# wangchen615/kubernetes-simulator

Measured on AMD Instinct MI355X. Metric: pod-node Filter+Score evals/sec and pods bound/sec at 50k nodes, 1-8 GPUs, higher is better.
Workload: dtype int64; 1 GPU; C3: 50k nodes w/ taints+labels, 1M-pod trace, Filter(fit+taint+selector) -> Score(LR+BA) -> argmax -> bind, 1 pod/tick; nodes=50000, trace_pods=5570560, parallelism=single-gpu, batch_pods=192

## Files before the change

go/kubesim/engine/engine.go:

```go
package engine

import "C"

import (
	"runtime"
	"unsafe"

	"github.com/cpuguy83/strongerrors"
	"github.com/pkg/errors"
)

var ErrOutOfDomain = errors.New("outside the engine's exact domain")

type Engine struct {
	h *C.ks_engine
	n int
}

func status(e *Engine, rc C.ks_status) error {
	msg := ""
	if e != nil && e.h != nil {
		msg = C.GoString(C.ks_last_error(e.h))
	}
	switch rc {
	case C.KS_OK:
		return nil
	case C.KS_ENOTFOUND:
		return strongerrors.NotFound(errors.New(msg))
	case C.KS_EINVAL:
		return strongerrors.InvalidArgument(errors.New(msg))
	case C.KS_ERANGE:
		return errors.Wrap(ErrOutOfDomain, msg)
	default:
		return errors.Errorf("ks_engine: device error (%d): %s", int(rc), msg)
	}
}

const (
	ScorerConst          = C.KS_SCORER_CONST
	ScorerLeastRequested = C.KS_SCORER_LEAST_REQUESTED
	ScorerBalanced       = C.KS_SCORER_BALANCED
)

const (
	FilterFit      = uint32(C.KS_FILTER_FIT)
	FilterTaint    = uint32(C.KS_FILTER_TAINT)
	FilterSelector = uint32(C.KS_FILTER_SELECTOR)
)

const (
	FlagNoOverlap   = uint32(C.KS_ENGINE_NO_OVERLAP)
	FlagPrunedLists = uint32(C.KS_ENGINE_PRUNED_LISTS)
)

type ScorerSpec struct {
	Kind, Weight, Value int32
}

type Config struct {
	TickSeconds int
	FeedsScore  bool
	Filters     uint32
	Scorers     []ScorerSpec
	Device      int
	BatchPods   int
	EngineFlags uint32
}

func (c Config) toC() (C.ks_config, error) {
	var cfg C.ks_config
	if len(c.Scorers) > 8 {
		return cfg, strongerrors.InvalidArgument(errors.New("at most 8 scorers"))
	}
	cfg.abi_version = C.KS_ABI_VERSION
	cfg.tick_seconds = C.int32_t(c.TickSeconds)
	if c.FeedsScore {
		cfg.filter_mode = C.KS_FILTER_FEEDS_SCORE
	}
	cfg.filters = C.uint32_t(c.Filters)
	cfg.n_scorers = C.int32_t(len(c.Scorers))
	for i, s := range c.Scorers {
		cfg.scorers[i].kind = C.int32_t(s.Kind)
		cfg.scorers[i].weight = C.int32_t(s.Weight)
		cfg.scorers[i].value = C.int32_t(s.Value)
	}
	cfg.device = C.int32_t(c.Device)
	cfg.batch_pods = C.int32_t(c.BatchPods)
	cfg.engine_flags = C.uint32_t(c.EngineFlags)
	return cfg, nil
}

func New(c Config) (*Engine, error) {
	cfg, err := c.toC()
	if err != nil {
		return nil, err
	}
	e := &Engine{}
	if rc := C.ks_create(&cfg, &e.h); rc != C.KS_OK {
		return nil, errors.Errorf("ks_create rejected the configuration (%d)", int(rc))
	}
	runtime.SetFinalizer(e, (*Engine).Close)
	return e, nil
}

func (e *Engine) Close() {
	if e.h != nil {
		C.ks_destroy(e.h)
		e.h = nil
	}
	runtime.SetFinalizer(e, nil)
}

func CommUniqueID() ([]byte, error) {
	id := make([]byte, C.KS_COMM_ID_BYTES)
	if rc := C.ks_comm_unique_id((*C.uint8_t)(unsafe.Pointer(&id[0]))); rc != C.KS_OK {
		return nil, status(nil, rc)
	}
	return id, nil
}

func (e *Engine) Shard(world, rank int, id []byte, vshards int) error {
	defer runtime.KeepAlive(e)
	if len(id) != C.KS_COMM_ID_BYTES {
		return errors.Errorf("communicator id: %d bytes, want %d", len(id), C.KS_COMM_ID_BYTES)
	}
	rc := C.ks_shard(e.h, C.int32_t(world), C.int32_t(rank), (*C.uint8_t)(unsafe.Pointer(&id[0])), C.int32_t(vshards))
	return status(e, rc)
}

func (e *Engine) LoadNodes(alloc []int64, taint, label []uint64) error {
	defer runtime.KeepAlive(e)
	n := len(taint)
	if len(alloc) != 4*n || len(label) != n {
		return strongerrors.InvalidArgument(errors.New("LoadNodes: alloc must hold 4 values per node"))
	}
	if n == 0 {
		return status(e, C.ks_load_nodes(e.h, 0, nil, nil, nil))
	}
	err := status(e, C.ks_load_nodes(e.h, C.int64_t(n), (*C.int64_t)(unsafe.Pointer(&alloc[0])),
		(*C.uint64_t)(unsafe.Pointer(&taint[0])), (*C.uint64_t)(unsafe.Pointer(&label[0]))))
	if err == nil {
		e.n = n
	}
	return err
}

type Pods struct {
	Arrival  []int64
	Req      []int64
	KeyMask  []uint8
	Tol, Sel []uint64
	PhaseOff []int32
	PhaseSec []int32
	PhaseUse []int64
	Flags    []uint8
	Key      []int64
}

func i64p(s []int64) *C.int64_t {
	if len(s) == 0 {
		return nil
	}
	return (*C.int64_t)(unsafe.Pointer(&s[0]))
}
func u64p(s []uint64) *C.uint64_t {
	if len(s) == 0 {
		return nil
	}
	return (*C.uint64_t)(unsafe.Pointer(&s[0]))
}
func i32p(s []int32) *C.int32_t {
	if len(s) == 0 {
		return nil
	}
	return (*C.int32_t)(unsafe.Pointer(&s[0]))
}
func u8p(s []uint8) *C.uint8_t {
	if len(s) == 0 {
		return nil
	}
	return (*C.uint8_t)(unsafe.Pointer(&s[0]))
}

func (e *Engine) SubmitPods(p *Pods) error {
	defer runtime.KeepAlive(e)
	m := len(p.Arrival)
	if m == 0 {
		return nil
	}
	if len(p.Req) != 3*m || len(p.KeyMask) != m || len(p.Tol) != m || len(p.Sel) != m ||
		len(p.PhaseOff) != m+1 || len(p.Flags) != m || len(p.Key) != m ||
		int(p.PhaseOff[m]) > len(p.PhaseSec) || 3*int(p.PhaseOff[m]) > len(p.PhaseUse) {
		return strongerrors.InvalidArgument(errors.New("SubmitPods: inconsistent array lengths"))
	}
	return status(e, C.ks_submit_pods(e.h, C.int64_t(m), i64p(p.Arrival), i64p(p.Req), u8p(p.KeyMask),
		u64p(p.Tol), u64p(p.Sel), i32p(p.PhaseOff), i32p(p.PhaseSec), i64p(p.PhaseUse), u8p(p.Flags),
		i64p(p.Key)))
}

type Bind struct {
	Pod    int64
	Node   int32
	Status int32
	Tick   int64
}
// ... 140 lines not shown
```

include/ks_engine.h:

```cpp
#ifndef KS_ENGINE_H
#define KS_ENGINE_H
#include <stdint.h>

#ifdef __cplusplus
extern "C" {
#endif

#define KS_ABI_VERSION 2

typedef enum {
    KS_OK = 0,
    KS_EINVAL = 1,
    KS_ENOTFOUND = 2,
    KS_EDEVICE = 3,
    KS_ENOMEM = 4,
    KS_ERANGE = 5,
} ks_status;

enum { KS_FILTER_REFERENCE_LITERAL = 0, KS_FILTER_FEEDS_SCORE = 1 };
enum { KS_FILTER_FIT = 1, KS_FILTER_TAINT = 2, KS_FILTER_SELECTOR = 4 };
enum { KS_SCORER_CONST = 0, KS_SCORER_LEAST_REQUESTED = 1, KS_SCORER_BALANCED = 2 };
enum { KS_POD_OK = 0, KS_POD_OVER_CAPACITY = 1 };
enum { KS_PODFLAG_BAD_KEY = 1, KS_PODFLAG_BAD_SPEC = 2 };

typedef struct {
    int32_t kind;
    int32_t weight;
    int32_t value;
} ks_scorer;

typedef struct {
    int32_t abi_version;
    int32_t tick_seconds;
    int32_t filter_mode;
    uint32_t filters;
    int32_t n_scorers;
    ks_scorer scorers[8];
    int32_t device;
    int32_t batch_pods;
    uint32_t engine_flags;
    int32_t reserved[7];
} ks_config;

enum { KS_ENGINE_FORCE_WIDE = 1, KS_ENGINE_NO_TINY = 2, KS_ENGINE_NO_MICRO = 4,
       KS_ENGINE_ONE_POD_RESOLVER = 8, KS_ENGINE_CHUNK_RESOLVER = 64, KS_ENGINE_NO_OVERLAP = 256,
       KS_ENGINE_PRUNED_LISTS = 512 };

typedef struct {
    int64_t pod;
    int32_t node;
    int32_t status;
    int64_t tick;
} ks_bind;

typedef struct ks_engine ks_engine;

ks_status ks_create(const ks_config* cfg, ks_engine** out);
void ks_destroy(ks_engine* eng);

typedef struct ks_group ks_group;
ks_status ks_group_create(int32_t device, int32_t max_scenarios, ks_group** out);
void ks_group_destroy(ks_group* g);
ks_status ks_group_add(ks_group* g, const ks_config* cfg, ks_engine** out);
int32_t ks_group_size(const ks_group* g);

ks_status ks_shard_layout(int64_t n_nodes, int32_t world, int32_t vshards, int32_t* part_lo_out);
ks_status ks_merge_candidates(const uint64_t* cand_all, int32_t parts, int32_t B, uint64_t* out);
#define KS_COMM_ID_BYTES 128
ks_status ks_comm_unique_id(uint8_t* id_out );
ks_status ks_shard(ks_engine* eng, int32_t world, int32_t rank, const uint8_t* id, int32_t vshards);
typedef ks_status (*ks_allgather_fn)(void* user, int32_t rank, int32_t world, void* buf, int64_t bytes_per_rank);
ks_status ks_shard_host(ks_engine* eng, int32_t world, int32_t rank, int32_t vshards, ks_allgather_fn fn,
                        void* user);

ks_status ks_load_nodes(ks_engine* eng, int64_t n, const int64_t* alloc, const uint64_t* taint,
                        const uint64_t* label);

ks_status ks_submit_pods(ks_engine* eng, int64_t m, const int64_t* arrival_tick,
                         const int64_t* req, const uint8_t* keymask, const uint64_t* tol,
                         const uint64_t* sel, const int32_t* phase_off, const int32_t* phase_sec,
                         const int64_t* phase_use, const uint8_t* flags, const int64_t* key_id);

ks_status ks_step(ks_engine* eng, int64_t ticks, ks_bind* out, int64_t cap, int64_t* n_out);

ks_status ks_filter(ks_engine* eng, int64_t pod, uint8_t* mask_out);
ks_status ks_score(ks_engine* eng, int64_t pod, int64_t* score_out);

ks_status ks_usage(ks_engine* eng, int64_t* usage_out);

ks_status ks_usage_at(ks_engine* eng, int64_t t, int64_t* usage_out);

ks_status ks_usage_digest(ks_engine* eng, int64_t t_lo, int64_t t_hi, uint64_t* out);
uint64_t ks_node_mix(int64_t node);

ks_status ks_requested_at(ks_engine* eng, int64_t t, int64_t* out);
ks_status ks_filter_at(ks_engine* eng, int64_t pod, uint8_t* mask_out);
ks_status ks_score_at(ks_engine* eng, int64_t pod, int64_t* score_out);
#define KS_SERIES_COLS 7
ks_status ks_cluster_series(ks_engine* eng, int64_t t_lo, int64_t t_hi, int64_t* out);
ks_status ks_node_peaks(ks_engine* eng, int64_t t_lo, int64_t t_hi, int64_t* out);

ks_status ks_pod_lookup(ks_engine* eng, int32_t node, int64_t key_id, int64_t* pod_out);
ks_status ks_node_pods(ks_engine* eng, int32_t node, int64_t* pods_out, int64_t cap, int64_t* n_out);

enum { KS_PHASE_PENDING = 0, KS_PHASE_RUNNING = 1, KS_PHASE_SUCCEEDED = 2, KS_PHASE_FAILED = 3 };
typedef struct {
    int32_t phase;
    int32_t node;
    int64_t start_tick;
    int32_t total_seconds;
    int32_t pad;
} ks_pod_info;
ks_status ks_pod_status(ks_engine* eng, int64_t pod_lo, int64_t n, ks_pod_info* out);

int64_t ks_current_tick(const ks_engine* eng);
int32_t ks_tick_seconds(const ks_engine* eng);
int64_t ks_queued_pods(const ks_engine* eng);
const char* ks_last_error(const ks_engine* eng);

typedef struct {
    double step_ms;
    double scan_ms;
    double resolve_ms;
    int64_t launches;
    int64_t pods;
    double other_ms;
} ks_step_stats;
ks_status ks_last_step_stats(const ks_engine* eng, ks_step_stats* out);
typedef struct {
    double prep_ms, scan_ms, merge_ms, resolve_ms, fused_ms, part_ms, xchg_ms;
    int64_t prep_n, scan_n, merge_n, resolve_n, fused_n, xchg_n;
    double side_scan_ms, side_part_ms, side_xchg_ms, wait_ms;
    int64_t side_n;
    double usage_ms;
    int64_t usage_n, usage_pods;
} ks_kernel_stats;
ks_status ks_last_step_kernels(const ks_engine* eng, ks_kernel_stats* out);
ks_status ks_group_step(ks_group* g, int64_t ticks, ks_bind* out, int64_t cap, int64_t* n_out,
                        int32_t* status_out, ks_step_stats* stats);
ks_status ks_debug_counters(ks_engine* eng, int64_t* out32);
ks_status ks_debug_invariants(ks_engine* eng, int64_t* out4);
ks_status ks_debug_window(ks_engine* eng, void* out, int64_t cap, int64_t* size_out);
ks_status ks_debug_watch(ks_engine* eng, int64_t pod);
enum { KS_SELFTEST_LR_MICRO = 0 };
ks_status ks_selftest(int32_t device, int32_t test, int64_t* failures);
void ks_set_profiling(ks_engine* eng, int enable);
const char* ks_build_id(void);

#ifdef __cplusplus
}
#endif
#endif
```

kubernetes-simulator_amd/csrc/ks_cand.hip:

```cpp
#include <climits>

#include "ks_device.h"
#include "ks_prep.h"
#include "ks_scan.h"

namespace ks {
namespace sq {

constexpr int kR = kChR;
constexpr int kPrepThreads = 1024;
constexpr int kClBuf = 256;
static_assert(kR <= kWave, "one candidate per lane");
static_assert(kWinSlots <= kPrepThreads, "one window slot per prep thread");

__device__ __forceinline__ int32_t key_node(uint64_t key) { return (int32_t)(0xFFFFFFFFu - (uint32_t)key); }
__device__ __forceinline__ int32_t clamp32(int64_t v) { return (int32_t)(v > INT_MAX ? INT_MAX : v); }

template <typename T>
__device__ __forceinline__ const __attribute__((address_space(1))) T* cg(const T* p) {
    return (const __attribute__((address_space(1))) T*)p;
}

__global__ __launch_bounds__(kPrepThreads) void window_prep_kernel(const EngineArgs* __restrict__ A, int head, int spec,
                                                                    int slot) {
    const EngineArgs& a = A[0];
    __shared__ prep::PrepLDS L;
    prep::prep_body<kPrepThreads>(a, a.ctr[kCtrStart], a.ctr[kCtrEnd], a.ctr[kCtrErr], head, spec, slot, L);
}

#ifdef KS_MCL_DIAG
#define MDG_AT(I, T)                                                                      \
    do {                                                                                  \
        const uint64_t t_ = prep::pstamp();                                               \
        if (threadIdx.x == 0) atomicAdd((unsigned long long*)&a.ctr[(I)], t_ - (T));      \
        (T) = t_;                                                                         \
    } while (0)
using prep::pstamp;
#endif
constexpr int kRecWords = 12;
static_assert(kRecWords <= kRecDw, "record size");
constexpr int kSlotPending = -2;
static_assert(kSlotIds <= 65535, "slot ids in 16 bits");

__device__ __forceinline__ void put_rec(uint32_t* o, const NodeV& v) {
    o[0] = (uint32_t)v.ac; o[1] = (uint32_t)v.am; o[2] = (uint32_t)v.ag;
    o[3] = (uint32_t)clamp32(v.ap);
    o[4] = (uint32_t)v.rc; o[5] = (uint32_t)v.rm; o[6] = (uint32_t)v.rg;
    o[7] = (uint32_t)v.nr;
    o[8] = (uint32_t)v.taint; o[9] = (uint32_t)(v.taint >> 32); o[10] = (uint32_t)v.label; o[11] = (uint32_t)(v.label >> 32);
}

constexpr int kEPer = kEMax / 256;

static_assert(kTopLOverlap >= kTopL, "merged lists kept at the longest list length");
template <int kMode, int kLL>
__device__ __forceinline__ void cand_list(const EngineArgs& a, WinWS& ws, int i, const uint64_t* cand,
                                          const uint64_t* ek, int n_e) {
    static_assert(kLL >= kTopL && kLL <= kWave, "one list entry per lane");
    const int tid = threadIdx.x;
    PDG(uint64_t pt = pstamp();)
    __shared__ uint64_t buf[kClBuf];
    __shared__ int cnt;
    __shared__ uint64_t s_thr;
    __shared__ int s_full;
    if (tid == 0) cnt = 0;
    __syncthreads();
    if (tid < kWave) {
        const int lane = tid;
        const uint64_t x = lane < kLL ? cand[lane] : 0ull;
        const bool un = x != 0 && a.e_idx[key_node(x)] < 0;
        const uint64_t um = __ballot(un);
        const int rank = __popcll(um & ((1ull << lane) - 1ull));
        if (un && rank < kTopL) {
            const int pos = atomicAdd(&cnt, 1);
            if (pos < kClBuf) buf[pos] = x;
        }
        const uint64_t last = cand[kLL - 1];
        const bool enough = __popcll(um) >= kTopL;
        if (enough && un && rank == kTopL - 1) s_thr = x;
        if (!enough && lane == 0) s_thr = last != 0 ? last : 1ull;
        if (lane == 0) s_full = enough || last != 0;
    }
    __syncthreads();
    PDG(MDG_AT(9, pt);)
    const uint64_t thr = s_thr;
    const bool full = s_full != 0;
    for (int k = tid; k < n_e; k += blockDim.x)
        if (ek[k] != 0 && ek[k] >= thr) {
            const int pos = atomicAdd(&cnt, 1);
            if (pos < kClBuf) buf[pos] = ek[k];
        }
    __syncthreads();
    PDG(MDG_AT(10, pt);)
    const int c = cnt, n = c < kClBuf ? c : kClBuf;
    __shared__ uint64_t kept[kR];
    if (tid < n) {
        const uint64_t me = buf[tid];
        int r = 0;
        for (int u = 0; u < n; ++u) r += buf[u] > me;
        if (r < kR) kept[r] = me;
    }
    __syncthreads();
    PDG(MDG_AT(11, pt);)
    if (tid < kWave) {
        const int lane = tid;
        const bool valid = lane < (n < kR ? n : kR);
        const uint64_t me = valid ? kept[lane] : 0ull;
        const int32_t nd = key_node(me);
        NodeV rec{};
        int32_t eix = -1;
        if (valid) { rec = load_node(a.s, nd); eix = a.e_idx[nd]; }
        if (valid && a.det_cids) atomicMin(&a.n_first[nd], i * kR + lane);
        int sl = valid ? atomicCAS(&a.n_slot[nd], -1, kSlotPending) : 0;
        const bool claim = valid && sl == -1;
        const uint64_t cm = __ballot(claim);
        int base = 0;
        if (cm) {
            const int first = __ffsll((unsigned long long)cm) - 1;
            if (lane == first) base = atomicAdd(&ws.nslot, __popcll(cm));
            base = __shfl(base, first);
        }
        if (claim) {
            sl = base + __popcll(cm & ((1ull << lane) - 1ull));
            ws.slot_node[sl] = nd;
            if (sl < kSlotMax) {
                put_rec(ws.slot_rec[sl], rec);
                ws.slot_eix[sl] = eix;
            }
            atomicExch(&a.n_slot[nd], sl);
        }
        bool wait = valid && sl == kSlotPending;
        while (__ballot(wait)) {
            if (wait) {
                sl = __hip_atomic_load(&a.n_slot[nd], __ATOMIC_RELAXED, __HIP_MEMORY_SCOPE_AGENT);
                wait = sl < 0;
            }
            if (__ballot(wait)) __builtin_amdgcn_s_sleep(1);
        }
        if (valid) {
            ws.cl_key[i][lane] = me;
            ws.cl_slot[i][lane] = sl;
        }
    }
    PDG(__syncthreads(); MDG_AT(12, pt);)
    if (tid == 0) {
        ws.cl_info[i] = (c < kR ? c : kR) | (c > kR ? kClTrunc : 0) | (full ? kClFull : 0) | (c > kClBuf ? kClOvf : 0);
        ws.cl_thr[i] = thr;
    }
}

constexpr int kMergeMaxWaves = 16;
}
#ifdef KS_MCL_BYVAL
thread_local const EngineArgs* ks_mcl_host_args = nullptr;
#endif
namespace sq {
template <int kMode, int kLL>
#ifdef KS_MCL_BYVAL
__global__ __launch_bounds__(1024) void merge_cl_kernel(const EngineArgs av, const uint64_t* src,
                                                         int64_t pod_stride, int32_t nl, int64_t list_stride, int own_fb) {
    const EngineArgs& a = av;
#else
__global__ __launch_bounds__(1024) void merge_cl_kernel(const EngineArgs* __restrict__ A, const uint64_t* src,
                                                         int64_t pod_stride, int32_t nl, int64_t list_stride, int own_fb) {
    const EngineArgs& a = A[0];
#endif
    WinWS& ws = *a.sw;
    const bool own = src == nullptr || (own_fb && ws.rescan);
    if (own) {
        src = a.lists;
        pod_stride = (int64_t)a.nblk * kLL;
        nl = a.nblk;
        list_stride = kLL;
    }
    const int b = blockIdx.x;
    const int tid = threadIdx.x, lane = tid & 63, wave = tid >> 6;
    const int nthr = blockDim.x, nwav = nthr / kWave;
    const bool prn = a.lbit != nullptr;
    const int lset = prn ? ws.lset : 1;
    const bool pruned = own && prn;
    const int nbw = ws.nb, split = ws.split, moff = ws.moff, mpar = ws.mpar;
    const bool reuse = b < split;
    const int sb = b - split;
    __shared__ scn::FlagLDS F;
    int nfl = reuse ? 0 : nl;
    if (b < nbw && !reuse && pruned) nfl = scn::flagged_index(lbit_of(a, lset, sb), 0, nl, F);
    if (prn) {
        const int cs = b < split ? nbw - split + b : (b < nbw ? sb : b);
        for (int w = tid; w < 2 * a.nwl; w += nthr) lbit_of(a, w / a.nwl, cs)[w % a.nwl] = 0;
        if (tid < 2 * kThrCopies) *lthr_of(a, tid / kThrCopies, tid % kThrCopies, cs) = 0;
    }
    if (b >= nbw) return;
    PDG(uint64_t pt = pstamp(); if (tid == 0) atomicAdd((unsigned long long*)&a.ctr[5], 1ull);)
    uint64_t top[kLL];
#pragma unroll
    for (int k = 0; k < kLL; ++k) top[k] = 0;
    const uint64_t* lists = src + (int64_t)(reuse ? 0 : sb) * pod_stride;
    uint64_t lv0[kLL];
    const bool has0 = tid < nfl;
    {
        const int l0 = has0 ? (pruned ? scn::flagged_block(tid, 0, nl, F) : tid) : 0;
        const ulonglong2* lp = reinterpret_cast<const ulonglong2*>(lists + (int64_t)l0 * list_stride);
#pragma unroll
        for (int k = 0; k < kLL / 2; ++k) {
            const ulonglong2 w = has0 ? lp[k] : make_ulonglong2(0, 0);
            lv0[2 * k] = w.x;
            lv0[2 * k + 1] = w.y;
        }
    }
    __shared__ uint64_t ek[kEMax];
    const int n_e = ws.n_e;
    {
        const int64_t start = a.ctr[kCtrStart];
        const int hi = ws.win_hi[b], n_es = ws.n_es;
        uint4 er[2][3];
        int32_t en[2], eu[2], ue[2];
#pragma unroll
        for (int q = 0; q < 2; ++q) {
            const int k = tid + q * nthr;
            const int kc = k < kEMax ? k : kEMax - 1;
            const int ks = k < kWinSlots ? k : kWinSlots;
            en[q] = ws.e_node[kc];
            const uint4* r = reinterpret_cast<const uint4*>(ws.e_rec[kc]);
            er[q][0] = r[0]; er[q][1] = r[1]; er[q][2] = r[2];
            eu[q] = ws.e_off[ks];
            ue[q] = ws.e_off[ks < kWinSlots ? ks + 1 : ks];
        }
#if defined(KS_MCL_DIAG) && KS_MCL_DIAG == 2
        asm volatile("s_waitcnt vmcnt(0) lgkmcnt(0)" ::: "memory");
        uint64_t t_e0 = pstamp();
        if (tid == 0) atomicAdd((unsigned long long*)&a.ctr[13], t_e0 - pt);
#endif
        const PodRec p = a.pods[start + b];
#pragma unroll
        for (int q = 0; q < 2; ++q) {
            const int k = tid + q * nthr;
            if (k >= n_e) continue;
            NodeV v = get_rec12(er[q]);
            if (k < n_es) {
                for (int u = eu[q]; u < ue[q]; ++u) {
                    const int x = ws.e_slot[u];
                    if (x >= hi) break;
                    v.rc -= ws.ex_req[x][0]; v.rm -= ws.ex_req[x][1]; v.rg -= ws.ex_req[x][2]; v.nr -= 1;
                }
            }
            ek[k] = make_key(eval_t<kMode>(a.c, p, v), (uint32_t)en[q]);
        }
#pragma unroll 1
        for (int k = tid + 2 * nthr; k < n_e; k += nthr) {
            const int32_t n = ws.e_node[k];
            const uint4* r = reinterpret_cast<const uint4*>(ws.e_rec[k]);
            const uint4 w3[3] = {r[0], r[1], r[2]};
            NodeV w = get_rec12(w3);
            const int ue1 = k < n_es ? ws.e_off[k + 1] : 0;
            for (int u = k < n_es ? ws.e_off[k] : 0; u < ue1; ++u) {
                const int x = ws.e_slot[u];
                if (x >= hi) break;
                w.rc -= ws.ex_req[x][0]; w.rm -= ws.ex_req[x][1]; w.rg -= ws.ex_req[x][2]; w.nr -= 1;
            }
            ek[k] = make_key(eval_t<kMode>(a.c, p, w), (uint32_t)n);
        }
#if defined(KS_MCL_DIAG) && KS_MCL_DIAG == 2
        asm volatile("s_waitcnt vmcnt(0) lgkmcnt(0)" ::: "memory");
        if (tid == 0) { atomicAdd((unsigned long long*)&a.ctr[14], pstamp() - t_e0); atomicAdd((unsigned long long*)&a.ctr[24], (unsigned long long)(n_e > tid) + (n_e > tid + nthr)); }
        if (tid == 0) atomicAdd((unsigned long long*)&a.ctr[25], (unsigned long long)n_e);
#endif
    }
    if (has0) {
#pragma unroll
        for (int k = 0; k < kLL; ++k) top[k] = lv0[k];
    }
    for (int j = tid + nthr; j < nfl; j += nthr) {
        const int blk = pruned ? scn::flagged_block(j, 0, nl, F) : j;
        const ulonglong2* lp = reinterpret_cast<const ulonglong2*>(lists + (int64_t)blk * list_stride);
        uint64_t lv[kLL];
#pragma unroll
        for (int k = 0; k < kLL / 2; ++k) {
            const ulonglong2 w = lp[k];
            lv[2 * k] = w.x;
            lv[2 * k + 1] = w.y;
        }
        topl_insert<kLL>(top, lv);
    }
    __shared__ uint64_t wl[kMergeMaxWaves][kLL];
    __shared__ uint64_t pc[kLL];
    PDG(MDG_AT(6, pt);)
    int head = 0;
    for (int r = 0; r < kLL; ++r) {
        uint64_t h = 0;
#pragma unroll
        for (int k = 0; k < kLL; ++k) h = (k == head) ? top[k] : h;
        const uint64_t m = wave_max_u64(h);
        const uint64_t hit = __ballot(h == m && m != 0);
        if (lane == 0) wl[wave][r] = m;
        if (hit && lane == __ffsll((unsigned long long)hit) - 1) head++;
    }
    __syncthreads();
    PDG(MDG_AT(7, pt);)
    if (wave == 0 && nthr <= 256) {
        static_assert(4 * kLL <= kWave, "one candidate per lane");
        uint64_t v = lane < nwav * kLL ? wl[lane / kLL][lane % kLL] : 0ull;
        for (int r = 0; r < kLL; ++r) {
            const uint64_t m = wave_max_u64(v);
            if (lane == 0) pc[r] = m;
            if (m == 0) continue;
            const uint64_t h = __ballot(v == m);
            if (lane == __ffsll((unsigned long long)h) - 1) v = 0;
        }
    } else if (wave == 0) {
        constexpr int kPer = (kMergeMaxWaves * kLL + kWave - 1) / kWave;
        const int nc = nwav * kLL;
        uint64_t v[kPer];
#pragma unroll
        for (int q = 0; q < kPer; ++q) {
            const int c = lane + q * kWave;
            v[q] = c < nc ? wl[c / kLL][c % kLL] : 0ull;
        }
        for (int r = 0; r < kLL; ++r) {
            uint64_t lm = v[0];
#pragma unroll
            for (int q = 1; q < kPer; ++q) lm = lm > v[q] ? lm : v[q];
            const uint64_t m = wave_max_u64(lm);
            if (lane == 0) pc[r] = m;
            if (m == 0) continue;
            bool done = false;
#pragma unroll
            for (int q = 0; q < kPer; ++q) {
                const uint64_t h = __ballot(!done && v[q] == m);
                if (h && lane == __ffsll((unsigned long long)h) - 1) v[q] = 0;
                done = done || h != 0;
            }
        }
    }
    __syncthreads();
    if (reuse && tid < kLL) pc[tid] = ws.mrg[mpar ^ 1][b + moff][tid];
    if (reuse) __syncthreads();
    if (tid < kLL) ws.mrg[mpar][b][tid] = pc[tid];
    PDG(MDG_AT(8, pt);)
    cand_list<kMode, kLL>(a, ws, b, pc, ek, n_e);
}

}

hipError_t launch_window_prep(const EngineArgs* d, bool head, bool spec, int slot, hipStream_t st) {
    hipLaunchKernelGGL(sq::window_prep_kernel, dim3(1), dim3(sq::kPrepThreads), 0, st, d, head ? 1 : 0, spec ? 1 : 0,
                       slot & 1);
    return hipGetLastError();
}

hipError_t launch_merge_cl(const EngineArgs* d, int mode, int B, const uint64_t* lists, int64_t pod_stride,
                           int32_t nl, int64_t list_stride, int nl_max, hipStream_t st, int L, bool own_fallback) {
    const int fb = own_fallback ? 1 : 0;
    static_assert(sq::kEPer * 256 >= kEMax, "E keys per thread at 256 threads");
    const dim3 g(B), t(nl_max > 1024 ? 1024 : 256);
#ifdef KS_MCL_BYVAL
    if (!ks_mcl_host_args) return hipErrorInvalidValue;
    const EngineArgs hv = *ks_mcl_host_args;
#define d hv
#endif
#define KS_MCL(LL)                                                                                                   \
    switch (mode) {                                                                                                  \
        case kEvalMicro: hipLaunchKernelGGL((sq::merge_cl_kernel<kEvalMicro, LL>), g, t, 0, st, d, lists, pod_stride, nl, list_stride, fb); break; \
        case kEvalTiny: hipLaunchKernelGGL((sq::merge_cl_kernel<kEvalTiny, LL>), g, t, 0, st, d, lists, pod_stride, nl, list_stride, fb); break;   \
        case kEvalNarrow: hipLaunchKernelGGL((sq::merge_cl_kernel<kEvalNarrow, LL>), g, t, 0, st, d, lists, pod_stride, nl, list_stride, fb); break; \
        default: hipLaunchKernelGGL((sq::merge_cl_kernel<kEvalWide, LL>), g, t, 0, st, d, lists, pod_stride, nl, list_stride, fb); break;          \
    }
    if (L == kTopL) { KS_MCL(kTopL) }
    else if (L == kTopLOverlap) { KS_MCL(kTopLOverlap) }
    else return hipErrorInvalidValue;
#undef KS_MCL
#ifdef KS_MCL_BYVAL
#undef d
#endif
    return hipGetLastError();
}

}
```

kubernetes-simulator_amd/csrc/ks_device.h:

```cpp
#pragma once
#include <hip/hip_runtime.h>
#include <stdint.h>

namespace ks {

constexpr int kWave = 64;
constexpr int kTopL = 8;
#ifndef KS_OVERLAP_LIST
#define KS_OVERLAP_LIST 12
#endif
constexpr int kTopLOverlap = KS_OVERLAP_LIST;
static_assert(kTopLOverlap >= kTopL && kTopLOverlap <= 16 && kTopLOverlap % 2 == 0, "overlap list length");

enum : uint32_t { kFilterFit = 1, kFilterTaint = 2, kFilterSelector = 4 };

struct Cfg {
    int32_t n_nodes;
    int32_t nwb;
    int32_t filter_feeds;
    uint32_t filters;
    int32_t has_scorers;
    int32_t w_lr;
    int32_t w_ba;
    int32_t const_total;
// ... 392 lines not shown

enum : int { kEvalWide = 0, kEvalNarrow = 1, kEvalTiny = 2, kEvalMicro = 3 };

template <int kMode, class NS>
__host__ __device__ __forceinline__ uint32_t eval_t(const Cfg& c, const PodRec& p, const NS& n) {
    if constexpr (kMode == kEvalMicro) return eval_total1_micro(c, p, n);
    else if constexpr (kMode == kEvalTiny) return eval_total1_tiny(c, p, n);
    else if constexpr (kMode == kEvalNarrow) return eval_total1_narrow(c, p, n);
    else return eval_total1(c, p, n);
}

constexpr float kBoundLR = 1.5e-5f;
constexpr float kBoundBA = 3.0e-5f;
struct PruneF {
    float bc, ic, bm, im;
    int32_t live;
};
template <class NS>
__host__ __device__ __forceinline__ PruneF prune_prep(const Cfg& c, const NS& n) {
    PruneF f;
    f.ic = n.ac > 0 ? rcp_est((float)n.ac) : 0.f;
    f.bc = n.ac > 0 ? (float)(int64_t)(n.ac - n.rc) * f.ic : -1.f;
    f.im = n.am > 0 ? rcp_est((float)n.am) : 0.f;
    f.bm = n.am > 0 ? (float)(int64_t)(n.am - n.rm) * f.im : -1.f;
    f.live = c.has_scorers && !(c.filter_feeds && (c.filters & kFilterFit) && n.nr >= n.ap);
    return f;
}
template <int kMode, class NS>
__host__ __device__ __forceinline__ PruneF prune_prep_t(const Cfg& c, const NS& n) {
    if constexpr (kMode >= kEvalNarrow) {
        const int32_t ac = (int32_t)n.ac, am = (int32_t)n.am;
        PruneF f;
        f.ic = ac > 0 ? rcp_est((float)ac) : 0.f;
        f.bc = ac > 0 ? (float)(ac - (int32_t)n.rc) * f.ic : -1.f;
        f.im = am > 0 ? rcp_est((float)am) : 0.f;
        f.bm = am > 0 ? (float)(am - (int32_t)n.rm) * f.im : -1.f;
        f.live = c.has_scorers && !(c.filter_feeds && (c.filters & kFilterFit) && n.nr >= n.ap);
        return f;
    } else {
        return prune_prep(c, n);
    }
}
__host__ __device__ __forceinline__ uint32_t prune_tmax(const Cfg& c, const PruneF& f, float qc, float qm) {
    const float fc = fmaf(-qc, f.ic, f.bc), fm = fmaf(-qm, f.im, f.bm);
    int32_t total = c.const_total;
    const int32_t lc = fc > -kBoundLR ? (int32_t)(10.f * fc + kBoundLR) : 0;
    const int32_t lm = fm > -kBoundLR ? (int32_t)(10.f * fm + kBoundLR) : 0;
    total += c.w_lr * ((lc + lm) >> 1);
    if (fc > -kBoundLR && fm > -kBoundLR)
        total += c.w_ba * (int32_t)(10.f - 10.f * fabsf(fc - fm) + kBoundBA);
    return (uint32_t)total;
}

template <typename T>
__device__ __forceinline__ T sload(const T* p) {
    static_assert(sizeof(T) % 4 == 0, "sload: dword-sized types only");
    typedef const __attribute__((address_space(4))) uint32_t* cp;
    const cp q = (cp)p;
    T v;
    uint32_t* d = reinterpret_cast<uint32_t*>(&v);
#pragma unroll
    for (int i = 0; i < (int)(sizeof(T) / 4); ++i) d[i] = q[i];
    return v;
}

template <typename T>
__device__ __forceinline__ __attribute__((address_space(1))) T* gptr(T* p) {
    return (__attribute__((address_space(1))) T*)p;
}

__host__ __device__ __forceinline__ uint64_t make_key(uint32_t total1, uint32_t node) {
    return total1 ? (((uint64_t)total1 << 32) | (uint64_t)(0xFFFFFFFFu - node)) : 0ull;
}

template <int L = kTopL>
__host__ __device__ __forceinline__ void topl_insert(uint64_t (&top)[L], const uint64_t (&lv)[L]) {
#pragma unroll
    for (int k = 0; k < L; ++k) {
        uint64_t v = lv[k];
        if (v <= top[L - 1]) break;
#pragma unroll
        for (int s = 0; s < L; ++s) {
            const uint64_t t = top[s];
            const bool gt = v > t;
            top[s] = gt ? v : t;
            v = gt ? t : v;
        }
    }
}

__device__ __forceinline__ uint32_t dpp_max_step(uint32_t v, uint32_t w) { return v > w ? v : w; }
__device__ __forceinline__ uint32_t wave_max_u32(uint32_t v) {
    v = dpp_max_step(v, (uint32_t)__builtin_amdgcn_update_dpp(0, (int)v, 0x111, 0xf, 0xf, false));
    v = dpp_max_step(v, (uint32_t)__builtin_amdgcn_update_dpp(0, (int)v, 0x112, 0xf, 0xf, false));
    v = dpp_max_step(v, (uint32_t)__builtin_amdgcn_update_dpp(0, (int)v, 0x114, 0xf, 0xf, false));
    v = dpp_max_step(v, (uint32_t)__builtin_amdgcn_update_dpp(0, (int)v, 0x118, 0xf, 0xf, false));
    v = dpp_max_step(v, (uint32_t)__builtin_amdgcn_update_dpp((int)v, (int)v, 0x142, 0xa, 0xf, false));
    v = dpp_max_step(v, (uint32_t)__builtin_amdgcn_update_dpp((int)v, (int)v, 0x143, 0xc, 0xf, false));
    return (uint32_t)__builtin_amdgcn_readlane((int)v, 63);
}

__device__ __forceinline__ uint64_t wave_max_u64(uint64_t v) {
    const uint32_t hi = (uint32_t)(v >> 32), lo = (uint32_t)v;
    const uint32_t mh = wave_max_u32(hi);
    const uint32_t ml = wave_max_u32(hi == mh ? lo : 0u);
    return ((uint64_t)mh << 32) | ml;
}

enum : int64_t { kCtrStart = 0, kCtrEnd = 1, kCtrErr = 2, kCtrErrPod = 3, kCtrEarly = 4, kCtrRescan = 5, kCtrReuse = 6 };
enum : uint32_t { kFlagBadKey = 1, kFlagBadSpec = 2 };
enum : int64_t { kErrEinval = 1, kErrNotFound = 2 };

constexpr int kWinMaxB = 256;
constexpr int kWinSlots = 512;
#ifndef KS_CHR
#define KS_CHR 20
#endif
constexpr int kChR = KS_CHR;
constexpr int kRecDw = 20;
constexpr int kSlotMax = 1536;
constexpr int kSlotIds = kWinMaxB * kChR;
constexpr int32_t kNoFirst = 0x7F7F7F7F;
constexpr int kEMax = 2048;
constexpr int kTouchMax = kWinMaxB + kWinSlots;
constexpr int kSpecStride = 8;
constexpr int kSpecPrev = 3;
enum : int32_t { kClTrunc = 1 << 8, kClFull = 1 << 9, kClOvf = 1 << 10 };
struct WinWS {
    int32_t nb, e_cnt, n_e, n_es;
    int32_t win_hi[kWinMaxB];
    int32_t own[kWinMaxB];
    int32_t ex_q[kWinSlots];
    int32_t ex_ok[kWinSlots];
    int64_t ex_req[kWinSlots][3];
    int32_t e_node[kEMax];
    int32_t e_off[kWinSlots + 1];
    int32_t e_slot[kWinSlots];
    uint32_t e_rec[kEMax][12];
    uint64_t cl_key[kWinMaxB][kChR];
    int32_t cl_info[kWinMaxB];
    uint64_t cl_thr[kWinMaxB];
    int32_t cl_slot[kWinMaxB][kChR];
    int32_t nslot;
    int32_t nslot_hw;
#ifdef KS_SLOT_IDS_LEGACY
    int32_t slot_node[kSlotMax];
#else
    int32_t slot_node[kSlotIds];
#endif
    int32_t slot_eix[kSlotMax];
    uint32_t slot_rec[kSlotMax][kRecDw];
    int32_t touched[kTouchMax];
    int32_t n_touched, rescan;
    int32_t lset, pad_;
    int32_t split, moff, mpar, pad2_;
    uint64_t mrg[2][kWinMaxB][kTopLOverlap];
#ifdef KS_BATCH_LOG
    int32_t blog_n, watch_pod, watch_done, wpad_;
    int32_t blog[16384][4];
    int32_t w_start, w_nb, w_c, w_n_e, w_n_es, w_pad[3];
    uint64_t w_cl_key[kWinMaxB][kChR];
    int32_t w_cl_info[kWinMaxB];
    uint64_t w_cl_thr[kWinMaxB];
    int32_t w_e_node[kEMax];
    int32_t w_bind[kWinMaxB];
    int32_t w_adm[kWinMaxB];
    int32_t w_nsw, w_pad2;
    int32_t w_dec[64][8];
    int16_t w_smeta[64][8];
    int32_t w_rowcid[64];
#endif
};

struct EngineArgs {
    Cfg c;
    NodeSoA s;
    const PodRec* pods;
    const int32_t* dur;
    const int64_t* exp_off;
    const int32_t* exp_pod;
    const int64_t* exp_pos;
    int32_t* b_node;
    int32_t* b_status;
    uint8_t* expired;
    uint64_t* lists;
    uint64_t* cand;
    int64_t* ctr;
    int32_t B;
    int32_t PG;
    int32_t nblk;
    int32_t blk_lo;
    int32_t blk_n;
    WinWS* sw;
    int32_t* e_idx;
    int32_t* n_slot;
    int32_t* n_first;
    int64_t* spec_ctr;
    uint64_t* lbit;
    uint64_t* lthr;
    int32_t nwl;
    int32_t lset;
    int32_t det_cids;
    int32_t pad3_;
    const ScanRec* srec;
};
__host__ __device__ __forceinline__ uint64_t* lbit_of(const EngineArgs& a, int set, int b) {
    return a.lbit + ((int64_t)set * a.B + b) * a.nwl;
}
constexpr int kThrCopies = 8;
__host__ __device__ __forceinline__ uint64_t* lthr_of(const EngineArgs& a, int set, int copy, int b) {
    return a.lthr + ((int64_t)set * kThrCopies + copy) * a.B + b;
}

int max_batch_pods();
int max_pods_per_scan_wg();
int block_nodes();
hipError_t launch_expire_head(const EngineArgs* d, int S, hipStream_t st);
hipError_t launch_scan(const EngineArgs* d, int S, int blk_n, int B, int PG, int mode, bool key16, hipStream_t st,
                       bool cond = false, bool prune = false, int L = kTopL, bool stage = false, int pw = 0);
hipError_t launch_merge(const EngineArgs* d, int S, int B, const uint64_t* lists, int64_t pod_stride, int32_t nl,
                        int64_t list_stride, uint64_t* out, int nl_max, hipStream_t st, const uint64_t* bits = nullptr,
                        int32_t nwl = 0, int32_t blk0 = 0, int32_t lset_fixed = -1, int L = kTopL);
hipError_t launch_resolve(const EngineArgs* d, int S, int mode, hipStream_t st);
hipError_t launch_resolve_small(const EngineArgs* d, int S, int mode, hipStream_t st);
int small_resolver_max_batch();
int small_resolver_max_nodes();
hipError_t launch_chunk_only(const EngineArgs* d, int mode, hipStream_t st);
hipError_t launch_chunk_scan(const EngineArgs* d, const EngineArgs* ds, int workers, int next_slot, int mode,
                             bool prune, int L, hipStream_t st);
hipError_t launch_window_prep(const EngineArgs* d, bool head, bool spec, int slot, hipStream_t st);
#ifdef KS_MCL_BYVAL
extern thread_local const EngineArgs* ks_mcl_host_args;
#endif
hipError_t launch_merge_cl(const EngineArgs* d, int mode, int B, const uint64_t* lists, int64_t pod_stride,
                           int32_t nl, int64_t list_stride, int nl_max, hipStream_t st, int L = kTopL,
                           bool own_fallback = false);
struct BindSeg {
    const int32_t* node;
    const int32_t* status;
    int64_t lo, n, off;
};
hipError_t launch_gather_binds(const BindSeg* segs, int S, int64_t max_n, int32_t* node, int32_t* status,
                               hipStream_t st);
hipError_t launch_rescale(const NodeSoA& s, int64_t n_pad, PodRec* pods, int64_t P, const int64_t f[3], hipStream_t st);

struct CopySeg {
    uint8_t* dst;
    const uint8_t* src;
    int64_t bytes;
};
hipError_t launch_scatter(const CopySeg* segs, int n, hipStream_t st);

constexpr int kTickMaxExp = 16;
struct TickExp {
    int32_t node, q;
    int64_t req[3];
};
struct TickScratch {
    uint64_t best;
    uint32_t count, pad_;
};
struct TickOut {
    int32_t node, status, code, pad_;
};
constexpr int kTickInl = 1024;
constexpr int kTickInlSeg = 32;
struct TickSeg {
    uint8_t* dst;
    int32_t off, bytes;
};
struct TickArgs {
    Cfg c;
    NodeSoA s;
    PodRec pod;
    int64_t j;
    int32_t run;
    int32_t n_exp;
    TickExp exp[kTickMaxExp];
    int32_t* b_node;
    int32_t* b_status;
    uint8_t* expired;
    TickScratch* scr;
    TickOut* out;
    int32_t n_iseg, pad_;
    TickSeg iseg[kTickInlSeg];
    alignas(16) uint8_t inl[kTickInl];
};
hipError_t launch_tick(const TickArgs& a, int mode, hipStream_t st);
struct ExpList {
    int32_t n, pad_;
    TickExp x[kTickMaxExp];
};
hipError_t launch_apply_exp(const NodeSoA& s, uint8_t* expired, const ExpList& l, hipStream_t st);
hipError_t launch_eval_pod(const Cfg& c, const NodeSoA& s, const PodRec* pod, uint32_t filters, uint8_t* mask,
                           int64_t* score, int mode, hipStream_t st);
hipError_t launch_flush(const NodeSoA& s, const PodRec* pods, const int64_t* fin, int64_t t, int64_t n_done,
                        const int32_t* b_node, const int32_t* b_status, uint8_t* expired, hipStream_t st);
hipError_t launch_selftest_lr_micro(unsigned long long* bad, hipStream_t st);
int usage_block_pods();
hipError_t launch_usage(const int32_t* blocks, int64_t nblocks, int64_t q_hi, int64_t t, int32_t tick_s,
                        const int32_t* b_node, const int32_t* b_status, const int64_t* t0, const int32_t* dur,
                        const int32_t* phase_off, const int32_t* cum_sec, const int64_t* use,
                        unsigned long long* usage, hipStream_t st);
hipError_t launch_usage_digest(const int32_t* blocks, int64_t nblocks, int64_t q_hi, int64_t t_lo, int64_t t_hi,
                               int32_t tick_s, const int32_t* b_node, const int32_t* b_status, const int64_t* t0,
                               const int32_t* dur, const uint8_t* preg, const int32_t* phase_off,
                               const int32_t* cum_sec, const int64_t* use, unsigned long long* diff,
                               unsigned long long* out, hipStream_t st);

struct QScale { int64_t f[3]; };
constexpr int kSeriesCols = 7;
struct SeriesInit { int64_t v[kSeriesCols]; };
hipError_t launch_requested(const int32_t* blocks, int64_t nblocks, int64_t q_hi, int64_t t, int32_t n_nodes,
                            const int32_t* b_node, const int32_t* b_status, const int64_t* t0, const int32_t* dur,
                            const PodRec* pods, const QScale& sc, int64_t node_stride, int64_t col_stride,
                            unsigned long long* out, hipStream_t st);
hipError_t launch_series(const int32_t* blocks, int64_t nblocks, int64_t q_lo, int64_t q_hi, int64_t t_lo,
                         int64_t t_hi, const int32_t* b_status, const int64_t* t0, const int32_t* dur,
                         const PodRec* pods, const QScale& sc, const int64_t* arr, int64_t n_arr,
                         const SeriesInit& init, unsigned long long* diff, unsigned long long* out, hipStream_t st);
hipError_t launch_node_peaks(const int32_t* blocks, int64_t nblocks, int64_t q_hi, int64_t t_lo, int32_t n_nodes,
                             const int32_t* b_node, const int32_t* b_status, const int64_t* t0, const int32_t* dur,
                             const PodRec* pods, const QScale& sc, int32_t* cnt, int32_t* off, int32_t* cur,
                             int32_t* list, int32_t list_cap, long long* out, hipStream_t st);

}
```

kubernetes-simulator_amd/csrc/ks_engine.cpp:

```cpp
#include <hip/hip_runtime.h>
#include <rccl/rccl.h>

#include <algorithm>
#include <cmath>
#include <numeric>
#include <cstdarg>
#include <cstdio>
#include <cstdlib>
#include <cstring>
#include <limits>
#include <queue>
#include <string>
#include <thread>
#include <unordered_map>
#include <vector>

#include "../../include/ks_engine.h"
#include "ks_device.h"


namespace {

constexpr int64_t kMaxNodes = 1LL << 24;
constexpr int64_t kMaxValue = 1LL << 59;
constexpr int kMaxBatch = 256;
constexpr int kDefaultBatch = 256;
constexpr int kChunkBatch = 192;
constexpr int64_t kStageMaxPods = 4096;
#ifndef KS_PG_MIN_WG
#define KS_PG_MIN_WG 2048
#endif
constexpr int kProfEv = 11;
constexpr int kRescanWgs = 1024;
constexpr int64_t kNever = std::numeric_limits<int64_t>::max();
constexpr int64_t kUBlk = 256;
constexpr int64_t kUSup = 64;
constexpr int64_t kMaxDigestTicks = 1 << 20;
#ifndef KS_OVERLAP_MAX_BLOCKS
#define KS_OVERLAP_MAX_BLOCKS 256
#endif
constexpr int kOverlapMaxBlocks = KS_OVERLAP_MAX_BLOCKS;

template <typename T>
struct DVec {
    T* p = nullptr;
    int64_t n = 0, cap = 0;
    hipError_t reserve(int64_t want, hipStream_t st) {
        if (want <= cap) return hipSuccess;
        int64_t nc = std::max<int64_t>(want, std::max<int64_t>(cap * 2, 1024));
        T* q = nullptr;
        hipError_t e = hipMalloc(&q, sizeof(T) * nc);
        if (e != hipSuccess) return e;
        if (n) {
            e = hipMemcpyAsync(q, p, sizeof(T) * n, hipMemcpyDeviceToDevice, st);
            if (e != hipSuccess) return e;
            e = hipStreamSynchronize(st);
            if (e != hipSuccess) return e;
        }
        if (p) (void)hipFree(p);
        p = q;
        cap = nc;
        return hipSuccess;
    }
    hipError_t append(const T* h, int64_t k, hipStream_t st) {
        hipError_t e = reserve(n + k, st);
        if (e != hipSuccess) return e;
        if (k) e = hipMemcpyAsync(p + n, h, sizeof(T) * k, hipMemcpyHostToDevice, st);
        n += k;
        return e;
    }
    void release() {
        if (p) (void)hipFree(p);
        p = nullptr;
        n = cap = 0;
    }
};

struct PendingHeap : std::priority_queue<std::pair<int64_t, int64_t>, std::vector<std::pair<int64_t, int64_t>>,
                                         std::greater<std::pair<int64_t, int64_t>>> {
    template <class F>
    void for_each_due(int64_t t, F&& f) const {
        std::vector<size_t> st;
        if (!c.empty() && c[0].first <= t) st.push_back(0);
        while (!st.empty()) {
            const size_t i = st.back();
            st.pop_back();
            f(c[i].second);
            for (size_t k = 2 * i + 1; k <= 2 * i + 2 && k < c.size(); k++)
                if (c[k].first <= t) st.push_back(k);
        }
    }
};

}

struct ks_engine {
    ks_config cfg{};
    ks::Cfg dc{};
    hipStream_t st = nullptr;
    int device = 0;
    bool profiling = false;

    int64_t n = 0, n_pad = 0;
    int nwb = 0;
    bool nodes_loaded = false;
    void* node_mem = nullptr;
    ks::NodeSoA s{};

    DVec<ks::PodRec> pods;
    DVec<int32_t> dur, b_node, b_status, phase_off, cum_sec, exp_pod;
    DVec<int64_t> exp_off, t0, fin, use, exp_pos;
    DVec<uint8_t> expired;
    DVec<ks::ScanRec> srec;
    std::vector<int64_t> h_bind_tick, h_fin;
    std::vector<int64_t> h_exp_off{0};
    std::vector<int32_t> h_dur;
    std::vector<int32_t> h_total_sec;
    PendingHeap pending;
    int64_t P = 0, F = 0;
    int64_t last_arrival = 0;
    int64_t scale[3] = {1, 1, 1};
    int64_t max_alloc[3] = {0, 0, 0};
    int mode = ks::kEvalWide;
    uint32_t flags = 0;
    std::vector<int64_t> h_exp_pos;
    std::vector<int64_t> h_key;
    std::unordered_map<int64_t, int64_t> key_end;
    std::vector<int32_t> h_node;
    std::vector<int8_t> h_status;
    std::vector<ks::PodRec> h_pods;
    std::vector<int32_t> h_exp_pod;
    std::vector<uint8_t> h_expired;
    uint8_t* stage = nullptr;
    uint8_t* stage_dev = nullptr;
    int64_t stage_cap = 0, stage_used = 0;
    ks::CopySeg* segs = nullptr;
    ks::CopySeg* segs_dev = nullptr;
    int seg_cap = 0, nseg = 0, seg_done = 0;
    int64_t xpos_lo = INT64_MAX;
    hipEvent_t stage_ev = nullptr;
    ks::TickScratch* d_tick = nullptr;
    ks::TickOut* h_tick = nullptr;
    ks::TickOut* h_tick_dev = nullptr;
    int64_t idx_upto = 0;
    std::vector<std::vector<int64_t>> node_pods;
    std::vector<int64_t> h_end, blk_end, sup_end;
    DVec<uint8_t> preg;

    int64_t tick = 0, done = 0;
    int err = KS_OK;
    std::string errmsg;

    int B = kDefaultBatch, PG = 32;
    uint64_t* lists = nullptr;
    uint64_t* cand = nullptr;
    int nblk = 0;
    int world = 1, rank = 0, vsh = 1;
    ncclComm_t comm = nullptr;
    ks_allgather_fn xfn = nullptr;
    void* xuser = nullptr;
    uint64_t* h_xbuf = nullptr;
    std::vector<int> part_lo;
    int blk_lo = 0, blk_n = 0;
    uint64_t* cand_all = nullptr;
    bool prune = false;
    int L = ks::kTopL;
    uint64_t* lbit = nullptr;
    uint64_t* lthr = nullptr;
    int nwl = 0;
    int64_t* d_ctr = nullptr;
    int64_t* h_ctr = nullptr;
    ks::EngineArgs* d_args = nullptr;
    ks::EngineArgs* h_args = nullptr;
    bool overlap = true;
    int scan_workers = 0;
    int64_t* d_spec = nullptr;
    ks::EngineArgs* d_args_spec = nullptr;
    ks::EngineArgs* h_args_spec = nullptr;
    hipStream_t st2 = nullptr;
    hipEvent_t pev_m = nullptr, pev_x = nullptr;
    ks::EngineArgs* d_args_full = nullptr;
    ks::EngineArgs* h_args_full = nullptr;
    ks_group* group = nullptr;
    hipEvent_t ev[4] = {nullptr, nullptr, nullptr, nullptr};
    std::vector<hipEvent_t> prof_ev;
    ks_step_stats stats{};
    ks_kernel_stats kstats{};

    uint8_t* d_mask = nullptr;
    int64_t* d_score = nullptr;
    ks::WinWS* d_sweep = nullptr;
    int32_t* d_eidx = nullptr;
    int32_t* d_nslot = nullptr;
    int32_t* d_first = nullptr;
    unsigned long long* d_usage = nullptr;
    DVec<int32_t> d_blk;
    std::vector<int32_t> h_blk;
    DVec<unsigned long long> d_digest;
    std::vector<int64_t> h_arr;
    std::vector<int64_t> cum_ok{0}, cum_over{0};
    int64_t cum_upto = 0;
    DVec<unsigned long long> d_qs;
    DVec<int32_t> d_qi;
};

namespace {

void engine_free(ks_engine* e);

bool in_passed_domain(const ks_engine* e, int64_t first_bind, int64_t t) {
    return t - first_bind <= (int64_t)INT32_MAX / e->cfg.tick_seconds;
}
ks_status fail(ks_engine* e, ks_status code, const char* fmt, ...) {
    char buf[512];
    va_list ap;
    va_start(ap, fmt);
    vsnprintf(buf, sizeof buf, fmt, ap);
    va_end(ap);
    if (e) e->errmsg = buf;
    return code;
}

#define HIPCHK(e, expr)                                                                     \
    do {                                                                                    \
        hipError_t _r = (expr);                                                             \
        if (_r != hipSuccess)                                                               \
            return fail((e), KS_EDEVICE, "%s failed: %s", #expr, hipGetErrorString(_r));    \
    } while (0)

ks::EngineArgs make_args(ks_engine* e) {
    ks::EngineArgs a{};
    a.c = e->dc;
    a.s = e->s;
    a.pods = e->pods.p;
    a.dur = e->dur.p;
    a.exp_off = e->exp_off.p;
    a.exp_pod = e->exp_pod.p;
    a.exp_pos = e->exp_pos.p;
    a.b_node = e->b_node.p;
    a.b_status = e->b_status.p;
    a.expired = e->expired.p;
    a.lists = e->lists;
    a.cand = e->cand;
    a.nblk = e->nblk;
    a.blk_lo = e->blk_lo;
    a.blk_n = e->blk_n;
    a.ctr = e->d_ctr;
    a.B = e->B;
    a.PG = e->PG;
    a.sw = e->d_sweep;
    a.e_idx = e->d_eidx;
    a.n_slot = e->d_nslot;
    a.n_first = e->d_first;
    a.det_cids = e->world * e->vsh > 1 ? 1 : 0;
    a.spec_ctr = e->d_spec;
    a.lbit = e->prune ? e->lbit : nullptr;
    a.lthr = e->prune ? e->lthr : nullptr;
    a.nwl = e->nwl;
    a.lset = 1;
    a.srec = e->srec.p;
    return a;
}

hipError_t stage_copy(ks_engine* e, void* dst, const void* src, int64_t bytes);
hipError_t stage_xpos(ks_engine* e) {
    const int64_t lo = e->xpos_lo;
    if (lo >= e->P) return hipSuccess;
    e->xpos_lo = INT64_MAX;
    return stage_copy(e, e->exp_pos.p + lo, e->h_exp_pos.data() + lo, sizeof(int64_t) * (e->P - lo));
}

hipError_t stage_flush(ks_engine* e) {
    if (hipError_t r = stage_xpos(e); r != hipSuccess) return r;
    if (e->seg_done >= e->nseg) return hipSuccess;
    hipError_t r = ks::launch_scatter(e->segs_dev + e->seg_done, e->nseg - e->seg_done, e->st);
    if (r == hipSuccess) r = hipEventRecord(e->stage_ev, e->st);
    e->seg_done = e->nseg;
    return r;
}

hipError_t stage_room(ks_engine* e, int64_t bytes) {
    if (e->nseg > 0 && e->seg_done == e->nseg && hipEventQuery(e->stage_ev) == hipSuccess) {
        e->stage_used = 0;
        e->nseg = e->seg_done = 0;
    }
    const int64_t need = e->stage_used + bytes + 16;
    if (need <= e->stage_cap && e->nseg < e->seg_cap) return hipSuccess;
    hipError_t r = stage_flush(e);
    if (r == hipSuccess) r = hipStreamSynchronize(e->st);
    if (r != hipSuccess) return r;
    e->stage_used = 0;
    e->nseg = e->seg_done = 0;
    if (bytes + 16 > e->stage_cap) {
        if (e->stage) (void)hipHostFree(e->stage);
        e->stage = nullptr;
        e->stage_cap = std::max<int64_t>(bytes + 16, std::max<int64_t>(2 * e->stage_cap, 1 << 20));
        r = hipHostMalloc(&e->stage, e->stage_cap, hipHostMallocMapped);
        if (r == hipSuccess) r = hipHostGetDevicePointer((void**)&e->stage_dev, e->stage, 0);
        if (r != hipSuccess) { e->stage = nullptr; e->stage_cap = 0; return r; }
    }
    if (e->seg_cap == 0) {
        e->seg_cap = 1 << 16;
        r = hipHostMalloc(&e->segs, sizeof(ks::CopySeg) * e->seg_cap, hipHostMallocMapped);
        if (r == hipSuccess) r = hipHostGetDevicePointer((void**)&e->segs_dev, e->segs, 0);
        if (r == hipSuccess && !e->stage_ev) r = hipEventCreateWithFlags(&e->stage_ev, hipEventDisableTiming);
        if (r != hipSuccess) { e->seg_cap = 0; return r; }
    }
    return hipSuccess;
}

hipError_t stage_copy(ks_engine* e, void* dst, const void* src, int64_t bytes) {
    if (bytes <= 0) return hipSuccess;
    hipError_t r = stage_room(e, bytes);
    if (r != hipSuccess) return r;
    std::memcpy(e->stage + e->stage_used, src, bytes);
    e->segs[e->nseg++] = ks::CopySeg{(uint8_t*)dst, e->stage_dev + e->stage_used, bytes};
    e->stage_used += (bytes + 15) / 16 * 16;
    return hipSuccess;
}

template <typename T>
hipError_t stage_append(ks_engine* e, DVec<T>& v, const T* h, int64_t k) {
    if (v.n + k > v.cap) {
        hipError_t r = stage_flush(e);
        if (r == hipSuccess) r = v.reserve(v.n + k, e->st);
        if (r != hipSuccess) return r;
    }
    hipError_t r = stage_copy(e, v.p + v.n, h, sizeof(T) * k);
    v.n += k;
    return r;
}

bool key16(const ks_engine* e) {
    return (int64_t)e->dc.const_total + 10 * ((int64_t)e->dc.w_lr + e->dc.w_ba) + 1 < (1 << 16);
}

bool small_resolver(const ks_engine* e) {
    return e->B <= ks::small_resolver_max_batch() && e->dc.n_nodes <= ks::small_resolver_max_nodes();
}

bool chunk_eligible(const ks_engine* e) {
    bool words = e->mode >= ks::kEvalNarrow;
    if (!words) {
        words = true;
        for (int k = 0; k < 3; k++) words &= e->max_alloc[k] / e->scale[k] < (int64_t)0xFFFFFFFF;
    }
    return e->B <= ks::kWinMaxB && words && key16(e);
}
enum Resolver { kResolveRole = 0, kResolveSmall = 1, kResolveChunk = 4 };
int resolver_of(const ks_engine* e) {
    if ((e->flags & KS_ENGINE_CHUNK_RESOLVER) && chunk_eligible(e)) return kResolveChunk;
    if (e->flags & KS_ENGINE_ONE_POD_RESOLVER) return kResolveRole;
    if (small_resolver(e)) return kResolveSmall;
    return chunk_eligible(e) ? kResolveChunk : kResolveRole;
}
hipError_t launch_resolver(const ks::EngineArgs* d, int S, int mode, int which, hipStream_t st) {
    return which == kResolveSmall ? ks::launch_resolve_small(d, S, mode, st) : ks::launch_resolve(d, S, mode, st);
}
void update_mode(ks_engine* e) {
    int64_t m[3];
    for (int k = 0; k < 3; k++) m[k] = e->max_alloc[k] / e->scale[k];
    const bool narrow = m[0] < ks::kNarrowCap && m[1] < ks::kNarrowCap && m[2] < ks::kNarrowCap;
    const bool tiny = m[0] < ks::kTinyCap && m[1] < ks::kTinyCap && m[2] < ks::kTinyCap && m[0] * m[1] < ks::kTinyCap;
    const bool micro = m[0] < ks::kMicroCap && m[1] < ks::kMicroCap && m[2] < ks::kMicroCap &&
                       m[0] * m[1] < ks::kMicroProd && e->dc.w_lr < ks::kMicroWeight &&
                       e->dc.w_ba < ks::kMicroWeight;
    const bool no_tiny = (e->flags & KS_ENGINE_NO_TINY) != 0;
    e->mode = (e->flags & KS_ENGINE_FORCE_WIDE) ? ks::kEvalWide
            : (micro && !no_tiny && !(e->flags & KS_ENGINE_NO_MICRO)) ? ks::kEvalMicro
            : (tiny && !no_tiny) ? ks::kEvalTiny
            : narrow ? ks::kEvalNarrow : ks::kEvalWide;
}

}

extern "C" {

}

namespace {

ks_status engine_init(const ks_config* cfg, ks_engine** out) {
    if (!cfg || !out) return KS_EINVAL;
    *out = nullptr;
    if (cfg->abi_version != KS_ABI_VERSION) return KS_EINVAL;
    if (cfg->tick_seconds < 1) return KS_EINVAL;
    if (cfg->filter_mode != KS_FILTER_REFERENCE_LITERAL && cfg->filter_mode != KS_FILTER_FEEDS_SCORE)
        return KS_EINVAL;
    if (cfg->filters & ~7u) return KS_EINVAL;
    if (cfg->n_scorers < 0 || cfg->n_scorers > 8) return KS_EINVAL;
    if (cfg->batch_pods < 0 || cfg->batch_pods > kMaxBatch) return KS_EINVAL;
    if (cfg->engine_flags &
        ~(uint32_t)(KS_ENGINE_FORCE_WIDE | KS_ENGINE_NO_TINY | KS_ENGINE_NO_MICRO | KS_ENGINE_ONE_POD_RESOLVER |
                    KS_ENGINE_CHUNK_RESOLVER | KS_ENGINE_NO_OVERLAP | KS_ENGINE_PRUNED_LISTS))
        return KS_EINVAL;
    int64_t const_total = 0, w_lr = 0, w_ba = 0;
    for (int i = 0; i < cfg->n_scorers; i++) {
        const ks_scorer& sc = cfg->scorers[i];
        if (sc.weight < 0) return KS_EINVAL;
        switch (sc.kind) {
            case KS_SCORER_CONST:
                if (sc.value < 0) return KS_EINVAL;
                const_total += (int64_t)sc.weight * sc.value;
                break;
            case KS_SCORER_LEAST_REQUESTED: w_lr += sc.weight; break;
            case KS_SCORER_BALANCED: w_ba += sc.weight; break;
            default: return KS_EINVAL;
        }
    }
    if (const_total + 10 * (w_lr + w_ba) >= (1LL << 30) - 2) return KS_EINVAL;

    ks_engine* e = new ks_engine();
    e->cfg = *cfg;
    e->device = cfg->device;
    e->B = cfg->batch_pods ? cfg->batch_pods : kDefaultBatch;
    e->flags = cfg->engine_flags;
    e->overlap = !(cfg->engine_flags & KS_ENGINE_NO_OVERLAP);
    e->dc.filter_feeds = cfg->filter_mode == KS_FILTER_FEEDS_SCORE;
    e->dc.filters = cfg->filters;
    e->dc.has_scorers = cfg->n_scorers > 0;
    e->dc.w_lr = (int32_t)w_lr;
    e->dc.w_ba = (int32_t)w_ba;
    e->dc.const_total = (int32_t)const_total;
    e->dc.tick_seconds = cfg->tick_seconds;
    *out = e;
    return KS_OK;
}

}

extern "C" {

ks_status ks_create(const ks_config* cfg, ks_engine** out) {
    ks_engine* e = nullptr;
    const ks_status v = engine_init(cfg, &e);
    if (v != KS_OK) return v;
    hipError_t r = hipSetDevice(e->device);
    if (r == hipSuccess) r = hipStreamCreateWithFlags(&e->st, hipStreamNonBlocking);
    if (r == hipSuccess) r = hipMalloc(&e->d_ctr, 32 * sizeof(int64_t));
    if (r == hipSuccess) r = hipHostMalloc(&e->h_ctr, 32 * sizeof(int64_t), hipHostMallocDefault);
    if (r == hipSuccess) r = hipMalloc(&e->d_args, sizeof(ks::EngineArgs));
    if (r == hipSuccess) r = hipHostMalloc(&e->h_args, sizeof(ks::EngineArgs), hipHostMallocDefault);
    for (int i = 0; i < 4 && r == hipSuccess; i++) r = hipEventCreate(&e->ev[i]);
    if (r == hipSuccess) r = hipMemsetAsync(e->d_ctr, 0, 32 * sizeof(int64_t), e->st);
    if (r == hipSuccess) r = hipStreamSynchronize(e->st);
    if (r != hipSuccess) {
        engine_free(e);
        return KS_EDEVICE;
    }
    *out = e;
    return KS_OK;
}

}

namespace {

void engine_free(ks_engine* e) {
    if (!e) return;
    (void)hipSetDevice(e->device);
    if (e->st) (void)hipStreamSynchronize(e->st);
    e->pods.release(); e->dur.release(); e->b_node.release(); e->b_status.release();
    e->phase_off.release(); e->cum_sec.release(); e->exp_pod.release(); e->exp_off.release();
    e->t0.release(); e->fin.release(); e->use.release(); e->expired.release(); e->exp_pos.release();
    e->preg.release(); e->d_blk.release(); e->d_digest.release(); e->srec.release();
    e->d_qs.release(); e->d_qi.release();
    if (e->node_mem) (void)hipFree(e->node_mem);
    if (e->lists) (void)hipFree(e->lists);
    if (e->cand) (void)hipFree(e->cand);
    if (e->cand_all) (void)hipFree(e->cand_all);
    if (e->lbit) (void)hipFree(e->lbit);
    if (e->lthr) (void)hipFree(e->lthr);
    if (e->comm) (void)ncclCommDestroy(e->comm);
    if (e->h_xbuf) (void)hipHostFree(e->h_xbuf);
    if (!e->group) {
        if (e->d_ctr) (void)hipFree(e->d_ctr);
        if (e->h_ctr) (void)hipHostFree(e->h_ctr);
        if (e->d_args) (void)hipFree(e->d_args);
        if (e->h_args) (void)hipHostFree(e->h_args);
    }
    if (e->d_mask) (void)hipFree(e->d_mask);
    if (e->d_score) (void)hipFree(e->d_score);
    if (e->d_sweep) (void)hipFree(e->d_sweep);
    if (e->d_eidx) (void)hipFree(e->d_eidx);
    if (e->d_nslot) (void)hipFree(e->d_nslot);
    if (e->d_first) (void)hipFree(e->d_first);
    if (e->d_spec) (void)hipFree(e->d_spec);
    if (e->d_args_spec) (void)hipFree(e->d_args_spec);
    if (e->h_args_spec) (void)hipHostFree(e->h_args_spec);
    if (e->st2) (void)hipStreamSynchronize(e->st2);
    if (e->d_args_full) (void)hipFree(e->d_args_full);
    if (e->h_args_full) (void)hipHostFree(e->h_args_full);
    if (e->pev_m) (void)hipEventDestroy(e->pev_m);
    if (e->pev_x) (void)hipEventDestroy(e->pev_x);
    if (e->st2) (void)hipStreamDestroy(e->st2);
    if (e->d_usage) (void)hipFree(e->d_usage);
    if (e->stage) (void)hipHostFree(e->stage);
    if (e->segs) (void)hipHostFree(e->segs);
    if (e->stage_ev) (void)hipEventDestroy(e->stage_ev);
    if (e->d_tick) (void)hipFree(e->d_tick);
    if (e->h_tick) (void)hipHostFree(e->h_tick);
    for (auto ev : e->ev) if (ev) (void)hipEventDestroy(ev);
    for (auto ev : e->prof_ev) (void)hipEventDestroy(ev);
    if (e->st && !e->group) (void)hipStreamDestroy(e->st);
    delete e;
}

}

extern "C" {

void ks_destroy(ks_engine* e) {
    if (e && !e->group) engine_free(e);
}

ks_status ks_comm_unique_id(uint8_t* id_out) {
    if (!id_out) return KS_EINVAL;
    ncclUniqueId uid;
    if (ncclGetUniqueId(&uid) != ncclSuccess) return KS_EDEVICE;
    static_assert(sizeof(uid) == KS_COMM_ID_BYTES, "RCCL unique id size");
    std::memcpy(id_out, &uid, sizeof uid);
    return KS_OK;
}

ks_status ks_shard(ks_engine* e, int32_t world, int32_t rank, const uint8_t* id, int32_t vshards) {
    if (!e) return KS_EINVAL;
    if (e->nodes_loaded) return fail(e, KS_EINVAL, "ks_shard must precede ks_load_nodes");
    if (e->comm) return fail(e, KS_EINVAL, "already sharded");
    if (world < 1 || rank < 0 || rank >= world || vshards < 1 || (int64_t)world * vshards > 4096)
        return fail(e, KS_EINVAL, "bad shard geometry world=%d rank=%d vshards=%d", world, rank, vshards);
    if (world > 1 && !id) return fail(e, KS_EINVAL, "world > 1 needs a communicator id");
    HIPCHK(e, hipSetDevice(e->device));
    if (id) {
        ncclUniqueId uid;
        std::memcpy(&uid, id, sizeof uid);
        const ncclResult_t r = ncclCommInitRank(&e->comm, world, uid, rank);
        if (r != ncclSuccess) {
            e->comm = nullptr;
            return fail(e, KS_EDEVICE, "ncclCommInitRank: %s", ncclGetErrorString(r));
        }
    }
    e->world = world;
    e->rank = rank;
    e->vsh = vshards;
    return KS_OK;
}

ks_status ks_shard_host(ks_engine* e, int32_t world, int32_t rank, int32_t vshards, ks_allgather_fn fn, void* user) {
    if (!e) return KS_EINVAL;
    if (e->nodes_loaded) return fail(e, KS_EINVAL, "ks_shard_host must precede ks_load_nodes");
    if (e->comm || e->xfn) return fail(e, KS_EINVAL, "already sharded");
    if (!fn || world < 1 || rank < 0 || rank >= world || vshards < 1 || (int64_t)world * vshards > 4096)
        return fail(e, KS_EINVAL, "bad host-exchange shard geometry world=%d rank=%d vshards=%d", world, rank, vshards);
    e->world = world;
    e->rank = rank;
    e->vsh = vshards;
    e->xfn = fn;
    e->xuser = user;
    return KS_OK;
}

ks_status ks_merge_candidates(const uint64_t* cand_all, int32_t parts, int32_t B, uint64_t* out) {
    if (!cand_all || !out || parts < 1 || B < 0) return KS_EINVAL;
    constexpr int L = ks::kTopL;
    for (int64_t b = 0; b < B; b++) {
        uint64_t top[L] = {};
        for (int64_t p = 0; p < parts; p++) {
            uint64_t lv[L];
            std::memcpy(lv, cand_all + (p * B + b) * L, sizeof(lv));
            ks::topl_insert(top, lv);
        }
        std::memcpy(out + b * L, top, sizeof(top));
    }
    return KS_OK;
}

ks_status ks_shard_layout(int64_t n_nodes, int32_t world, int32_t vshards, int32_t* part_lo_out) {
    if (!part_lo_out || n_nodes < 0 || n_nodes > kMaxNodes || world < 1 || vshards < 1 || (int64_t)world * vshards > 4096)
        return KS_EINVAL;
    const int64_t n_pad = std::max<int64_t>(64, (n_nodes + 63) / 64 * 64);
    const int64_t nblk = (n_pad + ks::block_nodes() - 1) / ks::block_nodes();
    const int G = world * vshards;
    for (int p = 0; p <= G; p++) part_lo_out[p] = (int32_t)((int64_t)p * nblk / G);
    return KS_OK;
}

ks_status ks_load_nodes(ks_engine* e, int64_t n, const int64_t* alloc, const uint64_t* taint, const uint64_t* label) {
    if (!e) return KS_EINVAL;
    if (e->nodes_loaded) return fail(e, KS_EINVAL, "nodes already loaded");
    if (n < 0 || n > kMaxNodes) return fail(e, KS_EINVAL, "node count %lld outside [0, %lld]", (long long)n, (long long)kMaxNodes);
    if (n && (!alloc || !taint || !label)) return fail(e, KS_EINVAL, "null node buffer");
    for (int64_t i = 0; i < n; i++) {
        for (int k = 0; k < 3; k++)
            if (alloc[i * 4 + k] < -1 || alloc[i * 4 + k] >= kMaxValue)
                return fail(e, KS_EINVAL, "node %lld: capacity %d out of range", (long long)i, k);
        if (alloc[i * 4 + 3] < 0 || alloc[i * 4 + 3] >= kMaxValue)
            return fail(e, KS_EINVAL, "node %lld: pods capacity out of range", (long long)i);
    }
    HIPCHK(e, hipSetDevice(e->device));
    e->n = n;
    e->n_pad = std::max<int64_t>(64, (n + 63) / 64 * 64);
    e->nwb = (int)(e->n_pad / 64);
    const int64_t np = e->n_pad;
    for (int k = 0; k < 3; k++) {
        int64_t g = 0, mx = 0;
        for (int64_t i = 0; i < n; i++) {
            const int64_t v = alloc[i * 4 + k];
            if (v > 0) { g = std::gcd(g, v); mx = std::max(mx, v); }
        }
        e->scale[k] = g > 0 ? g : 1;
        e->max_alloc[k] = mx;
    }
    update_mode(e);
    std::vector<int64_t> h(10 * np, 0);
    for (int64_t i = 0; i < np; i++) {
        const bool real = i < n;
        for (int k = 0; k < 4; k++) h[k * np + i] = real ? alloc[i * 4 + k] : (k == 3 ? 0 : -1);
        for (int k = 0; k < 3; k++)
            if (real && h[k * np + i] > 0) h[k * np + i] /= e->scale[k];
        h[8 * np + i] = real ? (int64_t)taint[i] : 0;
        h[9 * np + i] = real ? (int64_t)label[i] : 0;
    }
    HIPCHK(e, hipMalloc(&e->node_mem, sizeof(int64_t) * 10 * np));
    HIPCHK(e, hipMemcpyAsync(e->node_mem, h.data(), sizeof(int64_t) * 10 * np, hipMemcpyHostToDevice, e->st));
    int64_t* b = (int64_t*)e->node_mem;
    e->s.ac = b; e->s.am = b + np; e->s.ag = b + 2 * np; e->s.ap = b + 3 * np;
    e->s.rc = b + 4 * np; e->s.rm = b + 5 * np; e->s.rg = b + 6 * np; e->s.nr = b + 7 * np;
    e->s.taint = (uint64_t*)(b + 8 * np); e->s.label = (uint64_t*)(b + 9 * np);
    e->dc.n_nodes = (int32_t)n;
    e->dc.nwb = e->nwb;
    e->nblk = (int)((e->n_pad + ks::block_nodes() - 1) / ks::block_nodes());
    const int G = e->world * e->vsh;
    e->part_lo.assign(G + 1, 0);
    (void)ks_shard_layout(n, e->world, e->vsh, e->part_lo.data());
    e->blk_lo = e->part_lo[e->rank * e->vsh];
    e->blk_n = e->part_lo[(e->rank + 1) * e->vsh] - e->blk_lo;
    if (!e->cfg.batch_pods && n < 16 * kDefaultBatch)
        e->B = (int)std::clamp<int64_t>(n / 16 / 32 * 32, 64, kDefaultBatch);
    if (!e->cfg.batch_pods && !e->group && !small_resolver(e) && chunk_eligible(e) &&
        !(e->flags & KS_ENGINE_ONE_POD_RESOLVER))
        e->B = kChunkBatch;
    int pg = 1;
    while (pg < ks::max_pods_per_scan_wg() && pg < e->B &&
           (int64_t)e->blk_n * ((e->B + pg * 2 - 1) / (pg * 2)) >= KS_PG_MIN_WG)
        pg *= 2;
    e->PG = pg;
    const int lmax = (G == 1 && e->blk_n <= kOverlapMaxBlocks) || G > 1 ? ks::kTopLOverlap : ks::kTopL;
    HIPCHK(e, hipMalloc(&e->lists, sizeof(uint64_t) * (size_t)e->B * e->nblk * lmax));
    HIPCHK(e, hipMalloc(&e->cand, sizeof(uint64_t) * (size_t)e->B * ks::kTopL));
    if (G > 1) HIPCHK(e, hipMalloc(&e->cand_all, sizeof(uint64_t) * (size_t)G * e->B * ks::kTopLOverlap));
    if (G > 1 && e->xfn) HIPCHK(e, hipHostMalloc(&e->h_xbuf, sizeof(uint64_t) * (size_t)G * e->B * ks::kTopLOverlap, hipHostMallocDefault));
    HIPCHK(e, hipMalloc(&e->d_mask, std::max<int64_t>(n, 1)));
    HIPCHK(e, hipMalloc(&e->d_score, sizeof(int64_t) * std::max<int64_t>(n, 1)));
    HIPCHK(e, hipMalloc(&e->d_usage, sizeof(unsigned long long) * 3 * std::max<int64_t>(n, 1)));
    HIPCHK(e, hipStreamSynchronize(e->st));
    e->nodes_loaded = true;
    return KS_OK;
}

ks_status ks_submit_pods(ks_engine* e, int64_t m, const int64_t* arrival, const int64_t* req, const uint8_t* keymask,
                         const uint64_t* tol, const uint64_t* sel, const int32_t* phase_off, const int32_t* phase_sec,
                         const int64_t* phase_use, const uint8_t* flags, const int64_t* key_id) {
    if (!e) return KS_EINVAL;
    if (!e->nodes_loaded) return fail(e, KS_EINVAL, "ks_load_nodes must precede ks_submit_pods");
    if (m < 0) return fail(e, KS_EINVAL, "negative pod count");
    if (m == 0) return KS_OK;
    if (!arrival || !req || !keymask || !tol || !sel || !phase_off) return fail(e, KS_EINVAL, "null pod buffer");
    if (e->P + m >= (1LL << 31)) return fail(e, KS_EINVAL, "too many pods");
    if (phase_off[0] != 0) return fail(e, KS_EINVAL, "phase_off[0] must be 0");
    const int64_t nf = phase_off[m];
    if (nf && (!phase_sec || !phase_use)) return fail(e, KS_EINVAL, "null phase buffer");
    int64_t last = e->last_arrival;
    for (int64_t i = 0; i < m; i++) {
        if (arrival[i] < last) return fail(e, KS_EINVAL, "arrival ticks must be non-decreasing (pod %lld)", (long long)(e->P + i));
        last = arrival[i];
        if (phase_off[i + 1] < phase_off[i]) return fail(e, KS_EINVAL, "phase_off must be non-decreasing");
        if (key_id && key_id[i] < 0) return fail(e, KS_EINVAL, "pod %lld: key ids must be >= 0", (long long)(e->P + i));
        for (int k = 0; k < 3; k++)
            if (req[i * 3 + k] < 0 || req[i * 3 + k] >= kMaxValue)
                return fail(e, KS_EINVAL, "pod %lld: request out of range", (long long)(e->P + i));
    }
    for (int64_t f = 0; f < nf * 3; f++)
        if (phase_use[f] < 0 || phase_use[f] >= kMaxValue) return fail(e, KS_EINVAL, "usage out of range");
    {
        int64_t pb = e->P ? e->h_bind_tick[e->P - 1] : e->tick;
        const int64_t first = e->P ? e->h_bind_tick[0] : std::max<int64_t>(pb + 1, std::max<int64_t>(arrival[0], e->tick + 1));
        for (int64_t i = 0; i < m; i++) {
            pb = std::max<int64_t>(pb + 1, std::max<int64_t>(arrival[i], e->tick + 1));
            if (!in_passed_domain(e, first, pb))
                return fail(e, KS_ERANGE, "pod %lld: bind tick %lld is %lld ticks after the first bind (tick %lld): "
                            "(t - t0) * %d s reaches 2^31 and Go's int32(passed seconds) leaves its domain",
                            (long long)(e->P + i), (long long)pb, (long long)(pb - first), (long long)first,
                            e->cfg.tick_seconds);
        }
    }
    std::unordered_map<int64_t, int64_t> new_end;
    if (key_id) {
        int64_t pb = e->P ? e->h_bind_tick[e->P - 1] : e->tick;
        for (int64_t i = 0; i < m; i++) {
            const int64_t bt = std::max<int64_t>(pb + 1, std::max<int64_t>(arrival[i], e->tick + 1));
            pb = bt;
            int64_t prev = std::numeric_limits<int64_t>::min();
            auto it = new_end.find(key_id[i]);
            if (it != new_end.end()) prev = it->second;
            else if (auto jt = e->key_end.find(key_id[i]); jt != e->key_end.end()) prev = jt->second;
            if (prev > bt)
                return fail(e, KS_ERANGE, "pod %lld: key %lld reused at bind tick %lld while an earlier pod with it may run "
                            "until tick %lld (Store would replace a running pod: outside the exact domain)",
                            (long long)(e->P + i), (long long)key_id[i], (long long)bt, (long long)prev);
            uint32_t acc = 0;
            for (int32_t f = phase_off[i]; f < phase_off[i + 1]; f++) acc += (uint32_t)phase_sec[f];
            const int32_t S = (int32_t)acc;
            const int64_t d = S > 0 ? ((int64_t)S + e->cfg.tick_seconds - 1) / e->cfg.tick_seconds : 0;
            new_end[key_id[i]] = std::max(prev, bt + d);
        }
    }

    {
        int64_t f[3] = {1, 1, 1};
        bool any = false;
        for (int k = 0; k < 3; k++) {
            int64_t g = e->scale[k];
            for (int64_t i = 0; i < m; i++)
                if ((keymask[i] >> k & 1) && req[i * 3 + k] > 0) g = std::gcd(g, req[i * 3 + k]);
            f[k] = e->scale[k] / g;
            any |= f[k] != 1;
            e->scale[k] = g;
        }
        if (any) {
            HIPCHK(e, hipSetDevice(e->device));
            HIPCHK(e, stage_flush(e));
            HIPCHK(e, ks::launch_rescale(e->s, e->n_pad, e->pods.p, e->P, f, e->st));
            HIPCHK(e, hipStreamSynchronize(e->st));
            for (ks::PodRec& r : e->h_pods)
                for (int k = 0; k < 3; k++) r.req[k] *= f[k];
            update_mode(e);
            if (e->P) {
                std::vector<ks::ScanRec> sr(e->P);
                for (int64_t q = 0; q < e->P; q++) sr[q] = ks::scan_rec_micro(e->dc, e->h_pods[q]);
                HIPCHK(e, hipMemcpy(e->srec.p, sr.data(), sizeof(ks::ScanRec) * e->P, hipMemcpyHostToDevice));
            }
        }
    }
    std::vector<ks::PodRec> recs(m);
    std::vector<ks::ScanRec> srecs(m);
    std::vector<int32_t> dur(m), poff(m), cum(nf);
    std::vector<int64_t> t0(m), fin(m), eoff(m);
    std::vector<int32_t> tsec(m);
    std::vector<int64_t> run_end(m);
    std::vector<int64_t> arr_eff(m);
    std::vector<uint8_t> reg(m);
    std::vector<int32_t> epod;
    epod.reserve(m);
    const int64_t epod_base = e->exp_pod.n;
    e->h_exp_pos.resize(e->P + m, -1);
    int64_t pos_lo = e->P;
    int64_t prev_bind = e->P ? e->h_bind_tick[e->P - 1] : e->tick;
    for (int64_t i = 0; i < m; i++) {
        const int64_t j = e->P + i;
        ks::PodRec& r = recs[i];
        const uint8_t km = keymask[i] & 7;
        for (int k = 0; k < 3; k++) r.req[k] = (km >> k & 1) ? req[i * 3 + k] / e->scale[k] : 0;
        r.tol = tol[i];
        r.sel = sel[i];
        r.keymask = km;
        r.flags = flags ? flags[i] : 0;
        srecs[i] = ks::scan_rec_micro(e->dc, r);
        const int64_t arr = std::max<int64_t>(arrival[i], e->tick + 1);
        const int64_t bt = std::max<int64_t>(prev_bind + 1, arr);
        prev_bind = bt;
        arr_eff[i] = arr;
        uint32_t acc = 0;
        int64_t acc64 = 0;
        bool nonneg = true;
        for (int32_t f = phase_off[i]; f < phase_off[i + 1]; f++) {
            acc += (uint32_t)phase_sec[f];
            acc64 += phase_sec[f];
// ... 262 lines not shown
    if (o.code < 0) { *rc = fail(e, KS_EDEVICE, "per-tick kernel wrote no result"); return true; }
    const int32_t node = o.node, status = o.status;
    *rc = step_finish(e, t_end, o.code ? j : j + 1, &node, &status, out, cap, n_out);
    e->stats.pods = *n_out;
    return true;
}

#ifndef KS_PRUNE_MIN_BLOCKS
#define KS_PRUNE_MIN_BLOCKS 1024
#endif
constexpr int kPruneMinBlocks = KS_PRUNE_MIN_BLOCKS;


static ks_status ensure_window_ws(ks_engine* e) {
    const int r = resolver_of(e);
    e->prune = r == kResolveChunk && !e->group && (e->nblk >= kPruneMinBlocks || (e->flags & KS_ENGINE_PRUNED_LISTS));
    if (e->prune && !e->lbit) {
        e->nwl = (e->nblk + 63) / 64;
        HIPCHK(e, hipMalloc(&e->lbit, sizeof(uint64_t) * 2 * (size_t)e->B * e->nwl));
        HIPCHK(e, hipMemsetAsync(e->lbit, 0, sizeof(uint64_t) * 2 * (size_t)e->B * e->nwl, e->st));
        HIPCHK(e, hipMalloc(&e->lthr, sizeof(uint64_t) * 2 * ks::kThrCopies * (size_t)e->B));
        HIPCHK(e, hipMemsetAsync(e->lthr, 0, sizeof(uint64_t) * 2 * ks::kThrCopies * (size_t)e->B, e->st));
    }
    if (e->d_sweep || r != kResolveChunk) return KS_OK;
    HIPCHK(e, hipMalloc(&e->d_sweep, sizeof(ks::WinWS)));
    HIPCHK(e, hipMemsetAsync(e->d_sweep, 0, sizeof(ks::WinWS), e->st));
    HIPCHK(e, hipMalloc(&e->d_eidx, sizeof(int32_t) * e->n_pad));
    HIPCHK(e, hipMemsetAsync(e->d_eidx, 0xFF, sizeof(int32_t) * e->n_pad, e->st));
    HIPCHK(e, hipMalloc(&e->d_nslot, sizeof(int32_t) * e->n_pad));
    HIPCHK(e, hipMemsetAsync(e->d_nslot, 0xFF, sizeof(int32_t) * e->n_pad, e->st));
    HIPCHK(e, hipMalloc(&e->d_first, sizeof(int32_t) * e->n_pad));
    HIPCHK(e, hipMemsetAsync(e->d_first, 0x7F, sizeof(int32_t) * e->n_pad, e->st));
    HIPCHK(e, hipMalloc(&e->d_spec, 2 * ks::kSpecStride * sizeof(int64_t)));
    HIPCHK(e, hipMemsetAsync(e->d_spec, 0, 2 * ks::kSpecStride * sizeof(int64_t), e->st));
    HIPCHK(e, hipMalloc(&e->d_args_spec, 2 * sizeof(ks::EngineArgs)));
    HIPCHK(e, hipHostMalloc(&e->h_args_spec, 2 * sizeof(ks::EngineArgs), hipHostMallocDefault));
    {
        int cus = 0;
        HIPCHK(e, hipDeviceGetAttribute(&cus, hipDeviceAttributeMultiprocessorCount, e->device));
#ifndef KS_SCAN_WORKERS_DIV
#define KS_SCAN_WORKERS_DIV 1
#endif
        e->scan_workers = std::max(15, cus / KS_SCAN_WORKERS_DIV - 1);
    }
    if (e->world * e->vsh > 1) {
        HIPCHK(e, hipStreamCreateWithFlags(&e->st2, hipStreamNonBlocking));
        HIPCHK(e, hipEventCreateWithFlags(&e->pev_m, hipEventDisableTiming));
        HIPCHK(e, hipEventCreateWithFlags(&e->pev_x, hipEventDisableTiming));
        HIPCHK(e, hipMalloc(&e->d_args_full, sizeof(ks::EngineArgs)));
        HIPCHK(e, hipHostMalloc(&e->h_args_full, sizeof(ks::EngineArgs), hipHostMallocDefault));
    }
    return KS_OK;
}

static hipError_t part_merges(ks_engine* e, const ks::EngineArgs* a, hipStream_t s, int lset_fixed) {
    const int64_t L = e->L, BL = (int64_t)e->B * L;
    for (int v = 0; v < e->vsh; v++) {
        const int p = e->rank * e->vsh + v;
        const int nlp = e->part_lo[p + 1] - e->part_lo[p];
        const hipError_t r = ks::launch_merge(a, 1, e->B, e->lists + (int64_t)e->part_lo[p] * L, (int64_t)e->nblk * L, nlp,
                                              L, e->cand_all + p * BL, nlp, s, e->prune ? e->lbit : nullptr, e->nwl,
                                              e->part_lo[p], lset_fixed, (int)L);
        if (r != hipSuccess) return r;
    }
    return hipSuccess;
}

static ks_status exchange(ks_engine* e, hipStream_t s) {
    const int64_t BL = (int64_t)e->B * e->L;
    if (e->comm) {
        const ncclResult_t nr = ncclAllGather(e->cand_all + (int64_t)e->rank * e->vsh * BL, e->cand_all,
                                              (size_t)e->vsh * BL, ncclUint64, e->comm, s);
        if (nr != ncclSuccess) return fail(e, KS_EDEVICE, "ncclAllGather: %s", ncclGetErrorString(nr));
    } else if (e->xfn) {
        const int64_t slice = (int64_t)e->vsh * BL, off = (int64_t)e->rank * slice;
        HIPCHK(e, hipMemcpyAsync(e->h_xbuf + off, e->cand_all + off, sizeof(uint64_t) * slice, hipMemcpyDeviceToHost, s));
        HIPCHK(e, hipStreamSynchronize(s));
        const ks_status xr = e->xfn(e->xuser, e->rank, e->world, e->h_xbuf, (int64_t)sizeof(uint64_t) * slice);
        if (xr != KS_OK) return fail(e, KS_EDEVICE, "host exchange failed (%d)", (int)xr);
        HIPCHK(e, hipMemcpyAsync(e->cand_all, e->h_xbuf, sizeof(uint64_t) * slice * e->world, hipMemcpyHostToDevice, s));
    }
    return KS_OK;
}

static ks_status pipe_batch(ks_engine* e, int64_t b, int64_t nbat, hipEvent_t* ev) {
    hipStream_t st = e->st, s2 = e->st2;
    const ks::EngineArgs* d = e->d_args;
    const int G = e->world * e->vsh;
    const int64_t L = e->L, BL = (int64_t)e->B * L;
    const bool first = b == 0, more = b + 1 < nbat;
    if (ev[0]) HIPCHK(e, hipEventRecord(ev[0], st));
    if (first) {
        HIPCHK(e, ks::launch_window_prep(d, true, false, (int)(b & 1), st));
        if (ev[1]) HIPCHK(e, hipEventRecord(ev[1], st));
        HIPCHK(e, ks::launch_scan(d, 1, e->blk_n, e->B, e->PG, e->mode, key16(e), st, false, e->prune, (int)L, true));
        if (ev[2]) HIPCHK(e, hipEventRecord(ev[2], st));
        HIPCHK(e, part_merges(e, d, st, -1));
        if (ev[5]) HIPCHK(e, hipEventRecord(ev[5], st));
        if (ks_status r = exchange(e, st); r != KS_OK) return r;
        if (ev[6]) HIPCHK(e, hipEventRecord(ev[6], st));
    } else {
        HIPCHK(e, hipStreamWaitEvent(st, e->pev_x, 0));
        if (ev[1]) HIPCHK(e, hipEventRecord(ev[1], st));
        HIPCHK(e, ks::launch_scan(e->d_args_full, 1, e->nblk, e->B, e->PG, e->mode, key16(e), st, true, e->prune, (int)L,
                                  true, kRescanWgs));
        if (ev[2]) HIPCHK(e, hipEventRecord(ev[2], st));
        if (ev[5]) HIPCHK(e, hipEventRecord(ev[5], st));
        if (ev[6]) HIPCHK(e, hipEventRecord(ev[6], st));
    }
    HIPCHK(e, ks::launch_merge_cl(d, e->mode, e->B, e->cand_all, L, G, BL, G, st, (int)L, !first));
    if (ev[3]) HIPCHK(e, hipEventRecord(ev[3], st));
    if (more) {
        HIPCHK(e, hipEventRecord(e->pev_m, st));
        HIPCHK(e, ks::launch_chunk_scan(d, e->d_args_spec + (b & 1), 0, (int)((b + 1) & 1), e->mode, e->prune, ks::kTopL, st));
    } else {
        HIPCHK(e, ks::launch_chunk_only(d, e->mode, st));
    }
    if (ev[4]) HIPCHK(e, hipEventRecord(ev[4], st));
    if (more) {
        const ks::EngineArgs* ds = e->d_args_spec + (b & 1);
        HIPCHK(e, hipStreamWaitEvent(s2, e->pev_m, 0));
        if (ev[7]) HIPCHK(e, hipEventRecord(ev[7], s2));
        HIPCHK(e, ks::launch_scan(ds, 1, e->blk_n, e->B, e->PG, e->mode, key16(e), s2, false, e->prune, (int)L, false));
        if (ev[8]) HIPCHK(e, hipEventRecord(ev[8], s2));
        HIPCHK(e, part_merges(e, ds, s2, 0));
        if (ev[9]) HIPCHK(e, hipEventRecord(ev[9], s2));
        if (ks_status r = exchange(e, s2); r != KS_OK) return r;
        if (ev[10]) HIPCHK(e, hipEventRecord(ev[10], s2));
        HIPCHK(e, hipEventRecord(e->pev_x, s2));
    }
    return KS_OK;
}

static ks_status step_body(ks_engine* e, int64_t ticks, ks_bind* out, int64_t cap, int64_t* n_out) {
    HIPCHK(e, hipSetDevice(e->device));
    if (ks_status r = ensure_window_ws(e); r != KS_OK) return r;
    const int64_t t_end = e->tick + ticks;
    int64_t p_hi = 0;
    if (!step_prepare(e, ticks, &p_hi)) {
        e->tick = t_end;
        return KS_OK;
    }
    if (p_hi == e->done + 1 && !e->group && e->world * e->vsh == 1 && e->n > 0 && !e->profiling &&
        !(e->flags & (KS_ENGINE_CHUNK_RESOLVER | KS_ENGINE_ONE_POD_RESOLVER))) {
        ks_status rc = KS_OK;
        if (tick_step(e, t_end, out, cap, n_out, &rc)) return rc;
    }
    const int64_t done0 = e->done;
    HIPCHK(e, stage_flush(e));
    hipStream_t st = e->st;
    const int which = resolver_of(e);
    const bool fused = which == kResolveChunk;
    HIPCHK(e, hipMemcpyAsync(e->d_ctr, e->h_ctr, 5 * sizeof(int64_t), hipMemcpyHostToDevice, st));
    HIPCHK(e, hipMemcpyAsync(e->d_args, e->h_args, sizeof(ks::EngineArgs), hipMemcpyHostToDevice, st));
    const bool overlap = fused && e->overlap && e->d_args_spec && key16(e) && e->blk_n <= kOverlapMaxBlocks;
    const bool pipe = fused && !overlap && e->overlap && e->st2 && e->world * e->vsh > 1;
    e->L = (overlap && e->world * e->vsh == 1 && !e->prune) || pipe ? ks::kTopLOverlap : ks::kTopL;
    if (pipe) {
        *e->h_args_full = *e->h_args;
        e->h_args_full->blk_lo = 0;
        e->h_args_full->blk_n = e->nblk;
        HIPCHK(e, hipMemcpyAsync(e->d_args_full, e->h_args_full, sizeof(ks::EngineArgs), hipMemcpyHostToDevice, st));
    }
    if (overlap || pipe) {
        for (int k = 0; k < 2; k++) {
            e->h_args_spec[k] = *e->h_args;
            e->h_args_spec[k].ctr = e->d_spec + ks::kSpecStride * k;
            e->h_args_spec[k].lset = 0;
        }
        HIPCHK(e, hipMemcpyAsync(e->d_args_spec, e->h_args_spec, 2 * sizeof(ks::EngineArgs), hipMemcpyHostToDevice, st));
    }
    HIPCHK(e, hipEventRecord(e->ev[0], st));
    const ks::EngineArgs* d = e->d_args;
#ifdef KS_MCL_BYVAL
    ks::ks_mcl_host_args = e->h_args;
#endif
    int64_t start = e->done;
    int64_t launches = 0;
    double scan_ms = 0, res_ms = 0;
    ks_kernel_stats ks{};
    std::vector<uint8_t> kind;
    while (true) {
        const int64_t nbat = (p_hi - start + e->B - 1) / e->B;
        for (int64_t b = 0; b < nbat; b++) {
            hipEvent_t ev[kProfEv] = {};
            if (e->profiling) {
                while ((int64_t)e->prof_ev.size() < kProfEv * (launches + 1)) {
                    hipEvent_t x;
                    HIPCHK(e, hipEventCreate(&x));
                    e->prof_ev.push_back(x);
                }
                for (int k = 0; k < kProfEv; k++) ev[k] = e->prof_ev[kProfEv * launches + k];
            }
            if (pipe) {
                ks_status pr = pipe_batch(e, b, nbat, ev);
                if (pr != KS_OK) return pr;
                if (e->profiling) kind.push_back((uint8_t)(8 | (b == 0 ? 1 : 0) | (b + 1 < nbat ? 2 : 0)));
                launches++;
                continue;
            }
            const bool spec = overlap && b > 0;
            if (ev[0]) HIPCHK(e, hipEventRecord(ev[0], st));
            if (!spec) HIPCHK(e, fused ? ks::launch_window_prep(d, true, false, (int)(b & 1), st) : ks::launch_expire_head(d, 1, st));
            if (ev[1]) HIPCHK(e, hipEventRecord(ev[1], st));
            HIPCHK(e, ks::launch_scan(d, 1, e->blk_n, e->B, e->PG, e->mode, key16(e), st, spec, e->prune, e->L, fused));
            if (ev[2]) HIPCHK(e, hipEventRecord(ev[2], st));
            const int G = e->world * e->vsh;
            hipEvent_t evx[2] = {ev[5], ev[6]};
            const int64_t L = ks::kTopL, BL = (int64_t)e->B * L;
            if (G == 1) {
                HIPCHK(e, fused ? ks::launch_merge_cl(d, e->mode, e->B, nullptr, 0, 0, 0, e->nblk, st, e->L)
                                : ks::launch_merge(d, 1, e->B, nullptr, 0, 0, 0, nullptr, e->nblk, st));
            } else {
                HIPCHK(e, part_merges(e, d, st, -1));
                if (evx[0]) HIPCHK(e, hipEventRecord(evx[0], st));
                if (ks_status r = exchange(e, st); r != KS_OK) return r;
                if (evx[1]) HIPCHK(e, hipEventRecord(evx[1], st));
                HIPCHK(e, fused ? ks::launch_merge_cl(d, e->mode, e->B, e->cand_all, L, G, BL, G, st)
                                : ks::launch_merge(d, 1, e->B, e->cand_all, L, G, BL, e->cand, G, st));
            }
            if (ev[3]) HIPCHK(e, hipEventRecord(ev[3], st));
            if (overlap && b + 1 < nbat)
                HIPCHK(e, ks::launch_chunk_scan(d, e->d_args_spec + (b & 1), e->scan_workers, (int)((b + 1) & 1), e->mode,
                                                e->prune, e->L, st));
            else
                HIPCHK(e, fused ? ks::launch_chunk_only(d, e->mode, st) : launch_resolver(d, 1, e->mode, which, st));
            if (ev[4]) HIPCHK(e, hipEventRecord(ev[4], st));
            if (e->profiling) kind.push_back((uint8_t)((!spec ? 1 : 0) | (overlap && b + 1 < nbat ? 2 : 0) | (G > 1 ? 4 : 0)));
            launches++;
        }
        HIPCHK(e, hipMemcpyAsync(e->h_ctr, e->d_ctr, 5 * sizeof(int64_t), hipMemcpyDeviceToHost, st));
        HIPCHK(e, hipStreamSynchronize(st));
        const int64_t prev = start;
        start = e->h_ctr[0];
        if (e->h_ctr[2] != 0 || start >= p_hi) break;
        if (start <= prev) return fail(e, KS_EDEVICE, "scheduling made no progress at pod %lld", (long long)start);
    }
    HIPCHK(e, hipEventRecord(e->ev[1], st));
    const int64_t new_done = start;
    const int64_t nb = new_done - e->done;
    std::vector<int32_t> node(nb), status(nb);
    if (nb) {
        HIPCHK(e, hipMemcpyAsync(node.data(), e->b_node.p + e->done, sizeof(int32_t) * nb, hipMemcpyDeviceToHost, st));
        HIPCHK(e, hipMemcpyAsync(status.data(), e->b_status.p + e->done, sizeof(int32_t) * nb, hipMemcpyDeviceToHost, st));
    }
    HIPCHK(e, hipStreamSynchronize(st));
    float ms = 0;
    (void)hipEventElapsedTime(&ms, e->ev[0], e->ev[1]);
    double other_ms = 0;
    if (e->profiling) {
        for (int64_t l = 0; l < launches; l++) {
            float t[4] = {};
            hipEvent_t* E = &e->prof_ev[kProfEv * l];
            if (kind[l] & 8) {
                float w = 0, sc = 0, pm = 0, xc = 0, mg = 0, rs = 0;
                (void)hipEventElapsedTime(&w, E[0], E[1]);
                (void)hipEventElapsedTime(&sc, E[1], E[2]);
                (void)hipEventElapsedTime(&pm, E[2], E[5]);
                (void)hipEventElapsedTime(&xc, E[5], E[6]);
                (void)hipEventElapsedTime(&mg, E[6], E[3]);
                (void)hipEventElapsedTime(&rs, E[3], E[4]);
                ks.wait_ms += w;
                ks.scan_ms += sc; ks.scan_n += 1; scan_ms += sc;
                ks.merge_ms += pm + xc + mg; ks.merge_n += 1; other_ms += pm + xc + mg + w;
                if (kind[l] & 1) { ks.part_ms += pm; ks.xchg_ms += xc; ks.xchg_n += 1; }
                if (kind[l] & 2) { ks.fused_ms += rs; ks.fused_n += 1; } else { ks.resolve_ms += rs; ks.resolve_n += 1; }
                res_ms += rs;
                if (kind[l] & 2) {
                    float a0 = 0, a1 = 0, a2 = 0;
                    (void)hipEventElapsedTime(&a0, E[7], E[8]);
                    (void)hipEventElapsedTime(&a1, E[8], E[9]);
                    (void)hipEventElapsedTime(&a2, E[9], E[10]);
                    ks.side_scan_ms += a0; ks.side_part_ms += a1; ks.side_xchg_ms += a2; ks.side_n += 1;
                }
                continue;
            }
            for (int k = 0; k < 4; k++) (void)hipEventElapsedTime(&t[k], E[k], E[k + 1]);
            if (kind[l] & 4) {
                float pm = 0, xc = 0;
                (void)hipEventElapsedTime(&pm, E[2], E[5]);
                (void)hipEventElapsedTime(&xc, E[5], E[6]);
                ks.part_ms += pm; ks.xchg_ms += xc;
                ks.xchg_n += 1;
            }
            other_ms += t[0] + t[2];
            scan_ms += t[1];
            res_ms += t[3];
            ks.prep_ms += t[0]; ks.prep_n += kind[l] & 1;
            ks.scan_ms += t[1]; ks.scan_n += 1;
            ks.merge_ms += t[2]; ks.merge_n += 1;
            if (kind[l] & 2) { ks.fused_ms += t[3]; ks.fused_n += 1; }
            else { ks.resolve_ms += t[3]; ks.resolve_n += 1; }
        }
    }
    e->kstats = ks;
    e->stats.step_ms = ms;
    e->stats.scan_ms = scan_ms;
    e->stats.resolve_ms = res_ms;
    e->stats.other_ms = other_ms;
    e->stats.launches = launches;
    e->stats.pods = nb;
    const ks_status rc = step_finish(e, t_end, new_done, node.data(), status.data(), out, cap, n_out);
    if (rc == KS_OK) mirror_expired(e, done0, e->done);
    return rc;
}

struct ks_group {
    int device = 0;
    int cap = 0;
    hipStream_t st = nullptr;
    std::vector<ks_engine*> engs;
    int64_t* d_ctr = nullptr;
    int64_t* h_ctr = nullptr;
    ks::EngineArgs* d_args = nullptr;
    ks::EngineArgs* h_args = nullptr;
    ks::BindSeg* d_seg = nullptr;
    ks::BindSeg* h_seg = nullptr;
    int32_t* d_out = nullptr;
    int32_t* h_out = nullptr;
    int64_t out_cap = 0;
    hipEvent_t ev[2] = {nullptr, nullptr};
    hipStream_t st2 = nullptr;
    hipEvent_t xev = nullptr;
    std::string errmsg;
};

ks_status ks_group_create(int32_t device, int32_t max_scenarios, ks_group** out) {
    if (!out || max_scenarios < 1 || max_scenarios > 65535) return KS_EINVAL;
    *out = nullptr;
    ks_group* g = new ks_group();
    g->device = device;
    g->cap = max_scenarios;
    hipError_t r = hipSetDevice(device);
    if (r == hipSuccess) r = hipStreamCreateWithFlags(&g->st, hipStreamNonBlocking);
    if (r == hipSuccess) r = hipStreamCreateWithFlags(&g->st2, hipStreamNonBlocking);
    if (r == hipSuccess) r = hipEventCreateWithFlags(&g->xev, hipEventDisableTiming);
    if (r == hipSuccess) r = hipMalloc(&g->d_ctr, sizeof(int64_t) * 32 * max_scenarios);
    if (r == hipSuccess) r = hipHostMalloc(&g->h_ctr, sizeof(int64_t) * 32 * max_scenarios, hipHostMallocDefault);
    if (r == hipSuccess) r = hipMalloc(&g->d_args, sizeof(ks::EngineArgs) * max_scenarios);
    if (r == hipSuccess) r = hipHostMalloc(&g->h_args, sizeof(ks::EngineArgs) * max_scenarios, hipHostMallocDefault);
    if (r == hipSuccess) r = hipMalloc(&g->d_seg, sizeof(ks::BindSeg) * max_scenarios);
    if (r == hipSuccess) r = hipHostMalloc(&g->h_seg, sizeof(ks::BindSeg) * max_scenarios, hipHostMallocDefault);
    for (int i = 0; i < 2 && r == hipSuccess; i++) r = hipEventCreate(&g->ev[i]);
    if (r == hipSuccess) r = hipMemsetAsync(g->d_ctr, 0, sizeof(int64_t) * 32 * max_scenarios, g->st);
    if (r == hipSuccess) r = hipStreamSynchronize(g->st);
    if (r != hipSuccess) {
        ks_group_destroy(g);
        return KS_EDEVICE;
    }
    *out = g;
    return KS_OK;
}

void ks_group_destroy(ks_group* g) {
    if (!g) return;
    (void)hipSetDevice(g->device);
    if (g->st) (void)hipStreamSynchronize(g->st);
    for (ks_engine* e : g->engs) engine_free(e);
    if (g->d_ctr) (void)hipFree(g->d_ctr);
    if (g->h_ctr) (void)hipHostFree(g->h_ctr);
    if (g->d_args) (void)hipFree(g->d_args);
    if (g->h_args) (void)hipHostFree(g->h_args);
    if (g->d_seg) (void)hipFree(g->d_seg);
    if (g->h_seg) (void)hipHostFree(g->h_seg);
    if (g->d_out) (void)hipFree(g->d_out);
    if (g->h_out) (void)hipHostFree(g->h_out);
    if (g->st2) (void)hipStreamSynchronize(g->st2);
    for (auto ev : g->ev) if (ev) (void)hipEventDestroy(ev);
    if (g->xev) (void)hipEventDestroy(g->xev);
    if (g->st2) (void)hipStreamDestroy(g->st2);
    if (g->st) (void)hipStreamDestroy(g->st);
    delete g;
}

ks_status ks_group_add(ks_group* g, const ks_config* cfg, ks_engine** out) {
    if (!g || !cfg || !out) return KS_EINVAL;
    *out = nullptr;
    if ((int)g->engs.size() >= g->cap) return KS_EINVAL;
    if (cfg->device != g->device) return KS_EINVAL;
    ks_engine* e = nullptr;
    const ks_status v = engine_init(cfg, &e);
    if (v != KS_OK) return v;
    const int idx = (int)g->engs.size();
    e->group = g;
    e->st = g->st;
    e->d_ctr = g->d_ctr + 32 * idx;
    e->h_ctr = g->h_ctr + 32 * idx;
    e->d_args = g->d_args + idx;
    e->h_args = g->h_args + idx;
    hipError_t r = hipSetDevice(g->device);
    for (int i = 0; i < 4 && r == hipSuccess; i++) r = hipEventCreate(&e->ev[i]);
    if (r != hipSuccess) {
        engine_free(e);
        return KS_EDEVICE;
    }
    g->engs.push_back(e);
    *out = e;
    return KS_OK;
}

int32_t ks_group_size(const ks_group* g) { return g ? (int32_t)g->engs.size() : -1; }

#ifndef KS_GROUP_SPLIT_MIN
#define KS_GROUP_SPLIT_MIN 64
#endif
constexpr int kGroupSplitMin = KS_GROUP_SPLIT_MIN;

ks_status ks_group_step(ks_group* g, int64_t ticks, ks_bind* out, int64_t cap, int64_t* n_out, int32_t* status_out,
                        ks_step_stats* stats) {
    if (!g || !n_out || !status_out || ticks < 0 || cap < 0) return KS_EINVAL;
    const int S = (int)g->engs.size();
    if (S == 0) return KS_OK;
    if (hipSetDevice(g->device) != hipSuccess) return KS_EDEVICE;
    std::vector<int64_t> p_hi(S, 0), t_end(S, 0);
    std::vector<char> live(S, 0), part(S, 0);
    int mode = ks::kEvalMicro, blk_n = 0, B = 0;
    bool k16 = true, small = true;
    for (ks_engine* e : g->engs) {
        B = std::max(B, e->B);
        k16 = k16 && key16(e);
        small = small && small_resolver(e);
    }
    const int which = small ? kResolveSmall : kResolveRole;
    int64_t blocks = 0;
    for (int i = 0; i < S; i++) {
        ks_engine* e = g->engs[i];
        n_out[i] = 0;
        status_out[i] = KS_OK;
        const bool out_of_domain = e->P > 0 && !in_passed_domain(e, e->h_bind_tick[0], e->tick + ticks);
        if (e->err || !e->nodes_loaded || e->world * e->vsh != 1 || out_of_domain) {
            status_out[i] = e->err ? e->err : out_of_domain ? KS_ERANGE : KS_EINVAL;
            if (!e->err) {
                if (out_of_domain) fail(e, KS_ERANGE, "step past 2^31 s after the first bind");
                else fail(e, KS_EINVAL, "group step needs loaded, unsharded nodes");
            }
            e->h_ctr[0] = e->h_ctr[1] = e->done;
            e->h_ctr[2] = 0;
            *e->h_args = e->nodes_loaded ? make_args(e) : ks::EngineArgs{};
            e->h_args->ctr = e->d_ctr;
            e->h_args->blk_n = 0;
            continue;
        }
// ... 597 lines not shown
```

kubernetes-simulator_amd/csrc/ks_kernels.hip:

```cpp
#include <algorithm>

#include "ks_device.h"
#include "ks_scan.h"

namespace ks {

constexpr int kScanWaves = 4;
constexpr int kBlockNodes = kScanWaves * kWave;
constexpr int kL = kTopL;
#ifndef KS_MAX_PG
#define KS_MAX_PG 32
#endif
constexpr int kMaxPG = KS_MAX_PG;
constexpr int kResolveThreads = 1024;
constexpr int kOwnerWave0 = 3;
#ifndef KS_WRITER_WAVE
#define KS_WRITER_WAVE 5
#endif
#ifndef KS_PRIO
#define KS_PRIO 0
#endif
constexpr int kWriterWave = KS_WRITER_WAVE;
template <int THREADS, int TMAX, int HASH_LOG2, int MAXB, int FBITS_LOG2>
struct RCfg {
// ... 871 lines not shown
                c_prev = c;
            }
        }
    } else {
        for (int64_t t = a0; t < a1; ++t) {
            const int32_t passed = (int32_t)((t - s) * tick_s);
            for (int32_t f = f0; f < f1; ++f)
                if (passed < cum_sec[f]) {
                    digest_add(diff, T1, t - t_lo, t - t_lo + 1, use + (int64_t)f * 3, w);
                    break;
                }
        }
    }
}

__global__ __launch_bounds__(1024) void digest_scan_kernel(const unsigned long long* __restrict__ diff, int64_t T,
                                                            unsigned long long* __restrict__ out) {
    __shared__ unsigned long long part[1024];
    const int k = blockIdx.x, tid = threadIdx.x;
    const unsigned long long* d = diff + (int64_t)k * (T + 1);
    const int64_t chunk = (T + 1023) / 1024, lo = min<int64_t>(T, tid * chunk), hi = min<int64_t>(T, lo + chunk);
    unsigned long long s = 0;
    for (int64_t i = lo; i < hi; ++i) s += d[i];
    part[tid] = s;
    __syncthreads();
    for (int off = 1; off < 1024; off <<= 1) {
        const unsigned long long v = tid >= off ? part[tid - off] : 0ull;
        __syncthreads();
        part[tid] += v;
        __syncthreads();
    }
    unsigned long long run = tid ? part[tid - 1] : 0ull;
    for (int64_t i = lo; i < hi; ++i) {
        run += d[i];
        out[i * 6 + k] = run;
    }
}

__global__ __launch_bounds__(256) void rescale_kernel(NodeSoA s, int64_t n_pad, PodRec* pods, int64_t P,
                                                      int64_t f0, int64_t f1, int64_t f2) {
    const int64_t stride = (int64_t)gridDim.x * blockDim.x;
    for (int64_t i = (int64_t)blockIdx.x * blockDim.x + threadIdx.x; i < n_pad; i += stride) {
        if (s.ac[i] >= 0) s.ac[i] *= f0;
        if (s.am[i] >= 0) s.am[i] *= f1;
        if (s.ag[i] >= 0) s.ag[i] *= f2;
        s.rc[i] *= f0; s.rm[i] *= f1; s.rg[i] *= f2;
    }
    for (int64_t q = (int64_t)blockIdx.x * blockDim.x + threadIdx.x; q < P; q += stride) {
        pods[q].req[0] *= f0; pods[q].req[1] *= f1; pods[q].req[2] *= f2;
    }
}

int max_batch_pods() { return kMaxBatchR; }
int max_pods_per_scan_wg() { return kMaxPG; }
int block_nodes() { return kBlockNodes; }

hipError_t launch_expire_head(const EngineArgs* d, int S, hipStream_t st) {
    hipLaunchKernelGGL(expire_head_kernel, dim3(S), dim3(256), 0, st, d);
    return hipGetLastError();
}

template <typename KT, bool kPrune, int kLL>
static void launch_scan_t(const EngineArgs* d, const dim3& g, size_t lds, int mode, int xcd, int cond, int stage, int pers,
                          hipStream_t st) {
    switch (mode) {
        case kEvalMicro: hipLaunchKernelGGL((scan_kernel<kEvalMicro, KT, kPrune, kLL>), g, dim3(kBlockNodes), lds, st, d, xcd, cond, stage, pers); break;
        case kEvalTiny: hipLaunchKernelGGL((scan_kernel<kEvalTiny, KT, kPrune, kLL>), g, dim3(kBlockNodes), lds, st, d, xcd, cond, stage, pers); break;
        case kEvalNarrow: hipLaunchKernelGGL((scan_kernel<kEvalNarrow, KT, kPrune, kLL>), g, dim3(kBlockNodes), lds, st, d, xcd, cond, stage, pers); break;
        default: hipLaunchKernelGGL((scan_kernel<kEvalWide, KT, kPrune, kLL>), g, dim3(kBlockNodes), lds, st, d, xcd, cond, stage, pers); break;
    }
}

hipError_t launch_scan(const EngineArgs* d, int S, int blk_n, int B, int PG, int mode, bool key16, hipStream_t st,
                       bool cond, bool prune, int L, bool stage, int pw) {
    if ((blk_n > 0 || (stage && S == 1)) && S > 0) {
        const int groups = (B + PG - 1) / PG;
        const size_t lds = (key16 ? sizeof(uint16_t) : sizeof(uint32_t)) * kBlockNodes * PG;
        const bool xcd = S == 1;
        int64_t wgs = std::max<int64_t>(((int64_t)blk_n * groups + 7) / 8 * 8, stage ? kStageWgs : 0);
        if (pw > 0 && S == 1) wgs = std::max<int64_t>(std::min<int64_t>(wgs, pw / 8 * 8), kStageWgs);
        const dim3 g = xcd ? dim3((unsigned)wgs, 1, 1) : dim3(blk_n, groups, S);
        const int x = xcd ? 1 : 0, c = cond ? 1 : 0, sg = stage && xcd ? 1 : 0;
        if (L != kTopL) {
            if (L != kTopLOverlap) return hipErrorInvalidValue;
            if (key16) {
                if (prune) launch_scan_t<uint16_t, true, kTopLOverlap>(d, g, lds, mode, x, c, sg, pw > 0 ? 1 : 0, st);
                else launch_scan_t<uint16_t, false, kTopLOverlap>(d, g, lds, mode, x, c, sg, pw > 0 ? 1 : 0, st);
            } else {
                if (prune) launch_scan_t<uint32_t, true, kTopLOverlap>(d, g, lds, mode, x, c, sg, pw > 0 ? 1 : 0, st);
                else launch_scan_t<uint32_t, false, kTopLOverlap>(d, g, lds, mode, x, c, sg, pw > 0 ? 1 : 0, st);
            }
        } else if (key16) {
            if (prune) launch_scan_t<uint16_t, true, kTopL>(d, g, lds, mode, x, c, sg, pw > 0 ? 1 : 0, st);
            else launch_scan_t<uint16_t, false, kTopL>(d, g, lds, mode, x, c, sg, pw > 0 ? 1 : 0, st);
        } else {
            if (prune) launch_scan_t<uint32_t, true, kTopL>(d, g, lds, mode, x, c, sg, pw > 0 ? 1 : 0, st);
            else launch_scan_t<uint32_t, false, kTopL>(d, g, lds, mode, x, c, sg, pw > 0 ? 1 : 0, st);
        }
    }
    return hipGetLastError();
}

hipError_t launch_merge(const EngineArgs* d, int S, int B, const uint64_t* lists, int64_t pod_stride, int32_t nl,
                        int64_t list_stride, uint64_t* out, int nl_max, hipStream_t st, const uint64_t* bits,
                        int32_t nwl, int32_t blk0, int32_t lset_fixed, int L) {
    const dim3 g(B, S), t(nl_max > 1024 ? 1024 : 256);
    if (L == kTopLOverlap && L != kTopL) {
        hipLaunchKernelGGL(merge_kernel<kTopLOverlap>, g, t, 0, st, d, lists, pod_stride, nl, list_stride, out, bits,
                           nwl, blk0, lset_fixed);
    } else if (L != kTopL) {
        return hipErrorInvalidValue;
    } else if ((int64_t)nl_max * kL <= kWave && !bits) {
        hipLaunchKernelGGL(merge_small_kernel, dim3((B + 3) / 4, S), dim3(256), 0, st, d, lists, pod_stride, nl,
                           list_stride, out);
    } else {
        hipLaunchKernelGGL(merge_kernel<kTopL>, g, t, 0, st, d, lists, pod_stride, nl, list_stride, out, bits, nwl, blk0,
                           lset_fixed);
    }
    return hipGetLastError();
}

template <class C>
static void launch_resolve_t(const EngineArgs* d, int S, int mode, hipStream_t st) {
    switch (mode) {
        case kEvalMicro: hipLaunchKernelGGL((resolve_kernel<kEvalMicro, C>), dim3(S), dim3(C::kThreads), 0, st, d); break;
        case kEvalTiny: hipLaunchKernelGGL((resolve_kernel<kEvalTiny, C>), dim3(S), dim3(C::kThreads), 0, st, d); break;
        case kEvalNarrow: hipLaunchKernelGGL((resolve_kernel<kEvalNarrow, C>), dim3(S), dim3(C::kThreads), 0, st, d); break;
        default: hipLaunchKernelGGL((resolve_kernel<kEvalWide, C>), dim3(S), dim3(C::kThreads), 0, st, d); break;
    }
}

hipError_t launch_resolve(const EngineArgs* d, int S, int mode, hipStream_t st) {
    launch_resolve_t<RBig>(d, S, mode, st);
    return hipGetLastError();
}

__global__ __launch_bounds__(256) void gather_binds_kernel(const BindSeg* __restrict__ segs, int32_t* node,
                                                            int32_t* status) {
    const BindSeg g = segs[blockIdx.y];
    for (int64_t i = (int64_t)blockIdx.x * blockDim.x + threadIdx.x; i < g.n; i += (int64_t)gridDim.x * blockDim.x) {
        node[g.off + i] = g.node[g.lo + i];
        status[g.off + i] = g.status[g.lo + i];
    }
}

hipError_t launch_gather_binds(const BindSeg* segs, int S, int64_t max_n, int32_t* node, int32_t* status,
                               hipStream_t st) {
    if (S <= 0 || max_n <= 0) return hipSuccess;
    const unsigned bx = (unsigned)std::min<int64_t>((max_n + 255) / 256, 64);
    hipLaunchKernelGGL(gather_binds_kernel, dim3(bx, S), dim3(256), 0, st, segs, node, status);
    return hipGetLastError();
}

hipError_t launch_rescale(const NodeSoA& s, int64_t n_pad, PodRec* pods, int64_t P, const int64_t f[3], hipStream_t st) {
    hipLaunchKernelGGL(rescale_kernel, dim3(1024), dim3(256), 0, st, s, n_pad, pods, P, f[0], f[1], f[2]);
    return hipGetLastError();
}

hipError_t launch_eval_pod(const Cfg& c, const NodeSoA& s, const PodRec* pod, uint32_t filters, uint8_t* mask,
                           int64_t* score, int mode, hipStream_t st) {
    const dim3 g((c.n_nodes + 255) / 256);
    switch (mode) {
        case kEvalMicro: hipLaunchKernelGGL(eval_pod_kernel<kEvalMicro>, g, dim3(256), 0, st, c, s, pod, filters, mask, score); break;
        case kEvalTiny: hipLaunchKernelGGL(eval_pod_kernel<kEvalTiny>, g, dim3(256), 0, st, c, s, pod, filters, mask, score); break;
        case kEvalNarrow: hipLaunchKernelGGL(eval_pod_kernel<kEvalNarrow>, g, dim3(256), 0, st, c, s, pod, filters, mask, score); break;
        default: hipLaunchKernelGGL(eval_pod_kernel<kEvalWide>, g, dim3(256), 0, st, c, s, pod, filters, mask, score); break;
    }
    return hipGetLastError();
}

__global__ __launch_bounds__(256) void selftest_lr_micro_kernel(unsigned long long* bad) {
    const int32_t A = (int32_t)(blockIdx.x * blockDim.x + threadIdx.x) + 1;
    if (A >= kMicroCap) return;
    const float r = 10.f * rcp_est((float)A);
    unsigned long long nbad = 0;
    for (int32_t x = 0; x <= A; ++x) {
        const int64_t q = lr10_micro(x, r), y = 10ll * x;
        nbad += (q * A <= y && y < (q + 1) * A) ? 0ull : 1ull;
    }
    if (nbad) atomicAdd(bad, nbad);
}

hipError_t launch_selftest_lr_micro(unsigned long long* bad, hipStream_t st) {
    hipLaunchKernelGGL(selftest_lr_micro_kernel, dim3((unsigned)((kMicroCap + 255) / 256)), dim3(256), 0, st, bad);
    return hipGetLastError();
}

hipError_t launch_flush(const NodeSoA& s, const PodRec* pods, const int64_t* fin, int64_t t, int64_t n_done,
                        const int32_t* b_node, const int32_t* b_status, uint8_t* expired, hipStream_t st) {
    if (n_done <= 0) return hipSuccess;
    const int64_t blocks = std::min<int64_t>((n_done + 255) / 256, 2048);
    hipLaunchKernelGGL(flush_kernel, dim3((unsigned)blocks), dim3(256), 0, st, s, pods, fin, t, n_done, b_node,
                       b_status, expired);
    return hipGetLastError();
}

int usage_block_pods() { return kUsageBlk; }

hipError_t launch_usage(const int32_t* blocks, int64_t nblocks, int64_t q_hi, int64_t t, int32_t tick_s,
                        const int32_t* b_node, const int32_t* b_status, const int64_t* t0, const int32_t* dur,
                        const int32_t* phase_off, const int32_t* cum_sec, const int64_t* use,
                        unsigned long long* usage, hipStream_t st) {
    if (nblocks <= 0) return hipSuccess;
    hipLaunchKernelGGL(usage_kernel, dim3((unsigned)nblocks), dim3(kUsageBlk), 0, st, blocks, q_hi, t, tick_s, b_node,
                       b_status, t0, dur, phase_off, cum_sec, use, usage);
    return hipGetLastError();
}

hipError_t launch_usage_digest(const int32_t* blocks, int64_t nblocks, int64_t q_hi, int64_t t_lo, int64_t t_hi,
                               int32_t tick_s, const int32_t* b_node, const int32_t* b_status, const int64_t* t0,
                               const int32_t* dur, const uint8_t* preg, const int32_t* phase_off,
                               const int32_t* cum_sec, const int64_t* use, unsigned long long* diff,
                               unsigned long long* out, hipStream_t st) {
    if (nblocks > 0)
        hipLaunchKernelGGL(usage_digest_kernel, dim3((unsigned)nblocks), dim3(kUsageBlk), 0, st, blocks, q_hi, t_lo,
                           t_hi, tick_s, b_node, b_status, t0, dur, preg, phase_off, cum_sec, use, diff);
    hipLaunchKernelGGL(digest_scan_kernel, dim3(6), dim3(1024), 0, st, diff, t_hi - t_lo, out);
    return hipGetLastError();
}
}
```

kubernetes-simulator_amd/csrc/ks_prep.h:

```cpp
#pragma once
#include "ks_device.h"

namespace ks {
namespace prep {

constexpr int kEHashLog2 = 12, kEHash = 1 << kEHashLog2;

#ifdef KS_MCL_DIAG
__device__ __forceinline__ uint64_t pstamp() {
    uint64_t t;
    __builtin_amdgcn_sched_barrier(0);
    asm volatile("s_memtime %0\n\ts_waitcnt lgkmcnt(0)" : "=s"(t)::"memory");
    __builtin_amdgcn_sched_barrier(0);
    return t;
}
#define PDG(...) __VA_ARGS__
#define PDG_AT(I, T)                                                                      \
    do {                                                                                  \
        const uint64_t t_ = pstamp();                                                     \
        if (threadIdx.x == 0) atomicAdd((unsigned long long*)&a.ctr[16 + (I)], t_ - (T)); \
        (T) = t_;                                                                         \
    } while (0)
#else
#define PDG(...)
#define PDG_AT(I, T)
#endif
static_assert(2 * kEMax <= kEHash, "E hash load <= 1/2");

__device__ __forceinline__ uint32_t ehslot(int32_t n) { return ((uint32_t)n * 2654435761u) >> (32 - kEHashLog2); }

struct PrepLDS {
    int32_t hk[kEHash], hv[kEHash];
    int32_t cnt[kWinSlots], fill[kWinSlots];
    int32_t xn[kEMax];
    int64_t off[kWinMaxB];
    int32_t wsum[16];
    int32_t s_ne, s_nx;
};

template <int NT>
__device__ __forceinline__ void prep_body(const EngineArgs& a, int64_t start, int64_t end, int64_t err, int head,
                                          int spec, int slot, PrepLDS& L) {
    static_assert(kWinSlots <= NT && kWinMaxB <= NT, "one window slot and one pod per thread");
    static_assert(NT / 64 <= 16, "wave sums");
    WinWS& ws = *a.sw;
    const int tid = threadIdx.x;
    PDG(uint64_t pt = pstamp();)
    int64_t* const spec_out = a.spec_ctr + kSpecStride * slot;
    const int64_t* const spec_in = a.spec_ctr + kSpecStride * (slot ^ 1);
    int nb = (int)min<int64_t>(min<int64_t>(a.B, kWinMaxB), end - start);
    if (err != 0 || nb <= 0) {
        if (tid == 0) {
            ws.nb = 0; ws.e_cnt = 0; ws.n_e = 0; ws.n_es = 0; ws.rescan = 0; ws.lset = 1;
            ws.split = 0; ws.moff = 0; ws.mpar = slot;
            spec_out[kCtrStart] = end; spec_out[kCtrEnd] = end; spec_out[kCtrErr] = 0; spec_out[kSpecPrev] = start;
        }
        return;
    }
    const int64_t e0 = a.exp_off[start], e1 = a.exp_off[start + 1];
    const int64_t e_base = e1;
    const int64_t myoff = tid < nb ? a.exp_off[start + tid + 1] : 0;
    const int64_t mypos = tid < nb ? a.exp_pos[start + tid] : 0;
    const int64_t sp_start = spec ? spec_in[kCtrStart] : 0;
    const int64_t prev_start = spec ? spec_in[kSpecPrev] : 0;
    const int n_touched = spec ? ws.n_touched : 0;
    const int n_eold = spec ? ws.n_e : 0;
    constexpr int kOPer = (kEMax + NT - 1) / NT;
    int32_t eold[kOPer];
#pragma unroll
    for (int q = 0; q < kOPer; ++q) {
        const int t = tid + q * NT;
        eold[q] = spec && t < kEMax ? ws.e_node[t] : -1;
    }
    constexpr int kTPer = (kTouchMax + NT - 1) / NT;
    int32_t tch[kTPer];
#pragma unroll
    for (int q = 0; q < kTPer; ++q) {
        const int t = tid + q * NT;
        tch[q] = spec && t < kTouchMax ? ws.touched[t] : -1;
    }
    const bool fits_win = tid < nb && myoff - e_base <= kWinSlots;
    if (tid < nb) L.off[tid] = myoff;
    for (int h = tid; h < kEHash; h += NT) L.hk[h] = -1;
    if (tid == 0) { L.s_ne = 0; L.s_nx = 0; }
    nb = __syncthreads_count(fits_win);
    PDG_AT(0, pt);
    const int e_cnt = (int)(L.off[nb - 1] - e_base);
    const bool reuse = spec && start != sp_start && start > prev_start && start < sp_start;
    int rescan = 0;
    if (spec) rescan = (start != sp_start && !reuse) ||
                       (int64_t)e_cnt + (e1 - e0) + n_touched + (reuse ? n_eold : 0) > kEMax;
    const bool touch = spec && !rescan;
    const int32_t hq = head && tid < e1 - e0 ? a.exp_pod[e0 + tid] : -1;
    const int32_t wq = tid < e_cnt ? a.exp_pod[e_base + tid] : -1;
    int32_t hst = 1, hex = 1, hnd = 0, wst = 1, wex = 1, wnd = 0;
    int64_t hr0 = 0, hr1 = 0, hr2 = 0, wr0 = 0, wr1 = 0, wr2 = 0;
    if (hq >= 0) {
        hst = a.b_status[hq]; hex = a.expired[hq]; hnd = a.b_node[hq];
        const PodRec& p = a.pods[hq];
        hr0 = p.req[0]; hr1 = p.req[1]; hr2 = p.req[2];
    }
    if (wq >= 0) {
        wst = a.b_status[wq]; wex = a.expired[wq]; wnd = a.b_node[wq];
        const PodRec& p = a.pods[wq];
        wr0 = p.req[0]; wr1 = p.req[1]; wr2 = p.req[2];
    }
    if (head) {
        if (hq >= 0 && hst == 0 && !hex) {
            atomicAdd((unsigned long long*)&a.s.rc[hnd], (unsigned long long)(-hr0));
            atomicAdd((unsigned long long*)&a.s.rm[hnd], (unsigned long long)(-hr1));
            atomicAdd((unsigned long long*)&a.s.rg[hnd], (unsigned long long)(-hr2));
            atomicAdd((unsigned long long*)&a.s.nr[hnd], (unsigned long long)(-1ll));
            a.expired[hq] = 1;
            if (touch) L.xn[atomicAdd(&L.s_nx, 1)] = hnd;
        }
        for (int64_t e = e0 + NT + tid; e < e1; e += NT) {
            const int32_t q = a.exp_pod[e];
            if (a.b_status[q] != 0 || a.expired[q]) continue;
            const int32_t nd = a.b_node[q];
            const PodRec& p = a.pods[q];
            atomicAdd((unsigned long long*)&a.s.rc[nd], (unsigned long long)(-p.req[0]));
            atomicAdd((unsigned long long*)&a.s.rm[nd], (unsigned long long)(-p.req[1]));
            atomicAdd((unsigned long long*)&a.s.rg[nd], (unsigned long long)(-p.req[2]));
            atomicAdd((unsigned long long*)&a.s.nr[nd], (unsigned long long)(-1ll));
            a.expired[q] = 1;
            if (touch) L.xn[atomicAdd(&L.s_nx, 1)] = nd;
        }
    }
    if (touch) {
#pragma unroll
        for (int q = 0; q < kTPer; ++q)
            if (tid + q * NT < n_touched) L.xn[atomicAdd(&L.s_nx, 1)] = tch[q];
        if (reuse) {
#pragma unroll
            for (int q = 0; q < kOPer; ++q)
                if (tid + q * NT < n_eold) L.xn[atomicAdd(&L.s_nx, 1)] = eold[q];
        }
    }
    if (tid < nb) {
        ws.win_hi[tid] = tid >= 1 ? (int32_t)(myoff - e_base) : 0;
        ws.own[tid] = (mypos >= e_base && mypos - e_base < e_cnt) ? (int32_t)(mypos - e_base) : -1;
    }
    int32_t my_node = -1, my_k = -1;
    if (tid < e_cnt) {
        ws.ex_q[tid] = wq;
        ws.ex_req[tid][0] = wr0; ws.ex_req[tid][1] = wr1; ws.ex_req[tid][2] = wr2;
        const bool ok = wq < start && wst == 0 && !wex;
        ws.ex_ok[tid] = ok ? 1 : 0;
        if (ok) my_node = wnd;
    }
    if (my_node >= 0) {
        uint32_t h = ehslot(my_node);
        bool claimed = false;
        for (;;) {
            const int32_t prev = atomicCAS(&L.hk[h], -1, my_node);
            if (prev == -1) { claimed = true; break; }
            if (prev == my_node) break;
            h = (h + 1) & (kEHash - 1);
        }
        my_k = (int32_t)h;
        if (claimed) L.hv[h] = atomicAdd(&L.s_ne, 1);
    }
    __syncthreads();
    PDG_AT(1, pt);
    const int n_es = L.s_ne;
    __syncthreads();
    const int n_x = L.s_nx;
    for (int t = tid; t < n_x; t += NT) {
        const int32_t nd = L.xn[t];
        uint32_t h = ehslot(nd);
        for (;;) {
            const int32_t prev = atomicCAS(&L.hk[h], -1, nd);
            if (prev == -1) { const int k = atomicAdd(&L.s_ne, 1); L.hv[h] = k; ws.e_node[k] = nd; break; }
            if (prev == nd) break;
            h = (h + 1) & (kEHash - 1);
        }
    }
    __syncthreads();
    PDG_AT(2, pt);
    const int n_e = L.s_ne;
    if (tid < n_es) { L.cnt[tid] = 0; L.fill[tid] = 0; }
    __syncthreads();
    int k_of = -1;
    if (my_node >= 0) {
        k_of = L.hv[my_k];
        ws.e_node[k_of] = my_node;
        atomicAdd(&L.cnt[k_of], 1);
    }
    __syncthreads();
    PDG_AT(3, pt);
    {
        const int lane = tid & 63, wv = tid >> 6;
        const int v = tid < n_es ? L.cnt[tid] : 0;
        int incl = v;
#pragma unroll
        for (int o = 1; o < 64; o <<= 1) {
            const int u = __shfl_up(incl, o);
            if (lane >= o) incl += u;
        }
        if (lane == 63) L.wsum[wv] = incl;
        __syncthreads();
        int base = 0;
        for (int g = 0; g < wv; ++g) base += L.wsum[g];
        if (tid < n_es) ws.e_off[tid] = base + incl - v;
        if (tid == n_es - 1) ws.e_off[n_es] = base + incl;
        if (n_es == 0 && tid == 0) ws.e_off[0] = 0;
    }
    __syncthreads();
    PDG_AT(4, pt);
    if (my_node >= 0) ws.e_slot[ws.e_off[k_of] + atomicAdd(&L.fill[k_of], 1)] = tid;
    __syncthreads();
    PDG_AT(5, pt);
    if (tid < n_es) {
        const int lo = ws.e_off[tid], hi = ws.e_off[tid + 1];
        for (int u = lo + 1; u < hi; ++u) {
            const int32_t x = ws.e_slot[u];
            int v = u - 1;
            while (v >= lo && ws.e_slot[v] > x) { ws.e_slot[v + 1] = ws.e_slot[v]; --v; }
            ws.e_slot[v + 1] = x;
        }
    }
    for (int k = tid; k < n_e; k += NT) a.e_idx[ws.e_node[k]] = k;
    if (tid == 0) {
        ws.nb = nb; ws.e_cnt = e_cnt; ws.n_e = n_e; ws.n_es = n_es; ws.nslot = 0; ws.rescan = rescan;
        ws.lset = touch ? 0 : 1;
        if (rescan) a.ctr[kCtrRescan] += 1;
        if (touch && reuse) a.ctr[kCtrReuse] += 1;
        ws.split = touch && reuse ? (int32_t)(sp_start - start) : 0;
        ws.moff = (int32_t)(start - prev_start);
        ws.mpar = slot;
        spec_out[kCtrStart] = start + nb; spec_out[kCtrEnd] = end; spec_out[kCtrErr] = 0;
        spec_out[kSpecPrev] = start;
    }
    PDG(__syncthreads(); PDG_AT(6, pt); if (tid == 0) atomicAdd((unsigned long long*)&a.ctr[23], 1ull);)
}

}
}
```

kubernetes-simulator_amd/kubesim_amd/_lib.py:

```python
from __future__ import annotations

import ctypes as C
import os

HERE = os.path.dirname(os.path.abspath(__file__))
LIB_PATH = os.path.join(HERE, "libks_engine.so")
RUN_LIB_PATH = os.path.join(HERE, "libks_kubesim.so")

KS_OK, KS_EINVAL, KS_ENOTFOUND, KS_EDEVICE, KS_ENOMEM, KS_ERANGE = 0, 1, 2, 3, 4, 5
KS_FILTER_REFERENCE_LITERAL, KS_FILTER_FEEDS_SCORE = 0, 1
KS_FILTER_FIT, KS_FILTER_TAINT, KS_FILTER_SELECTOR = 1, 2, 4
KS_SCORER_CONST, KS_SCORER_LEAST_REQUESTED, KS_SCORER_BALANCED = 0, 1, 2
KS_POD_OK, KS_POD_OVER_CAPACITY = 0, 1
KS_PODFLAG_BAD_KEY, KS_PODFLAG_BAD_SPEC = 1, 2
KS_ABI_VERSION = 2
KS_ENGINE_FORCE_WIDE = 1
KS_ENGINE_NO_TINY = 2
KS_ENGINE_NO_MICRO = 4
KS_ENGINE_ONE_POD_RESOLVER = 8
KS_ENGINE_CHUNK_RESOLVER = 64
KS_ENGINE_NO_OVERLAP = 256
KS_ENGINE_PRUNED_LISTS = 512
KS_SELFTEST_LR_MICRO = 0
KS_SERIES_COLS = 7

STATUS_NAMES = {KS_OK: "OK", KS_EINVAL: "InvalidArgument", KS_ENOTFOUND: "NotFound",
                KS_EDEVICE: "DeviceError", KS_ENOMEM: "OutOfMemory", KS_ERANGE: "OutOfDomain"}

EXPORTED_SYMBOLS = ("ks_create", "ks_destroy", "ks_load_nodes", "ks_submit_pods", "ks_step",
                    "ks_filter", "ks_score", "ks_usage", "ks_current_tick", "ks_tick_seconds", "ks_queued_pods",
                    "ks_last_error", "ks_last_step_stats", "ks_last_step_kernels", "ks_set_profiling", "ks_debug_counters", "ks_debug_invariants", "ks_debug_window", "ks_debug_watch", "ks_build_id", "ks_selftest",
                    "ks_comm_unique_id", "ks_shard", "ks_shard_host", "ks_group_create", "ks_group_destroy",
                    "ks_group_add", "ks_group_size", "ks_group_step", "ks_pod_status",
                    "ks_usage_at", "ks_usage_digest", "ks_node_mix", "ks_pod_lookup", "ks_node_pods",
                    "ks_shard_layout", "ks_merge_candidates",
                    "ks_requested_at", "ks_filter_at", "ks_score_at", "ks_cluster_series", "ks_node_peaks",
                    "ks_parse_quantity", "ks_parse_simspec", "ks_cluster_parse", "ks_cluster_free",
                    "ks_cluster_nodes", "ks_cluster_tick", "ks_cluster_start_clock", "ks_cluster_arrays",
                    "ks_cluster_node_name", "ks_cluster_tolerations", "ks_cluster_selector",
                    "ks_cluster_parse_ex", "ks_cluster_note_pod", "ks_cluster_seal")
KS_CLUSTER_DEFER_MASKS = 1
KS_COMM_ID_BYTES = 128
RUN_SYMBOLS = ("ks_run", "ks_trace_submit", "ks_local_exchange_create", "ks_local_exchange_destroy",
               "ks_local_allgather", "ks_local_exchange_abort", "ks_run_build_id")


class KsScorer(C.Structure):
    _fields_ = [("kind", C.c_int32), ("weight", C.c_int32), ("value", C.c_int32)]


class KsConfig(C.Structure):
    _fields_ = [("abi_version", C.c_int32), ("tick_seconds", C.c_int32), ("filter_mode", C.c_int32),
                ("filters", C.c_uint32), ("n_scorers", C.c_int32), ("scorers", KsScorer * 8),
                ("device", C.c_int32), ("batch_pods", C.c_int32), ("engine_flags", C.c_uint32),
                ("reserved", C.c_int32 * 7)]


class KsBind(C.Structure):
    _fields_ = [("pod", C.c_int64), ("node", C.c_int32), ("status", C.c_int32), ("tick", C.c_int64)]


class KsPodInfo(C.Structure):
    _fields_ = [("phase", C.c_int32), ("node", C.c_int32), ("start_tick", C.c_int64),
                ("total_seconds", C.c_int32), ("pad", C.c_int32)]


KS_PHASE_PENDING, KS_PHASE_RUNNING, KS_PHASE_SUCCEEDED, KS_PHASE_FAILED = 0, 1, 2, 3


class KsStepStats(C.Structure):
    _fields_ = [("step_ms", C.c_double), ("scan_ms", C.c_double), ("resolve_ms", C.c_double),
                ("launches", C.c_int64), ("pods", C.c_int64), ("other_ms", C.c_double)]


class KsKernelStats(C.Structure):
    _fields_ = [("prep_ms", C.c_double), ("scan_ms", C.c_double), ("merge_ms", C.c_double),
                ("resolve_ms", C.c_double), ("fused_ms", C.c_double), ("part_ms", C.c_double),
                ("xchg_ms", C.c_double), ("prep_n", C.c_int64), ("scan_n", C.c_int64), ("merge_n", C.c_int64),
                ("resolve_n", C.c_int64), ("fused_n", C.c_int64), ("xchg_n", C.c_int64),
                ("side_scan_ms", C.c_double), ("side_part_ms", C.c_double), ("side_xchg_ms", C.c_double),
                ("wait_ms", C.c_double), ("side_n", C.c_int64),
                ("usage_ms", C.c_double), ("usage_n", C.c_int64), ("usage_pods", C.c_int64)]


class KsPods(C.Structure):
    _fields_ = [("m", C.c_int64), ("arrival", C.c_void_p), ("req", C.c_void_p), ("keymask", C.c_void_p),
                ("tol", C.c_void_p), ("sel", C.c_void_p), ("phase_off", C.c_void_p), ("phase_sec", C.c_void_p),
                ("phase_use", C.c_void_p), ("flags", C.c_void_p), ("key_id", C.c_void_p)]


class KsTraceSubmitter(C.Structure):
    _fields_ = [("trace", KsPods), ("next", C.c_int64), ("tick_seconds", C.c_int64)]


_lib = None
_run_lib = None
CSRC = os.path.join(os.path.dirname(HERE), "csrc")


def source_hash():
    import hashlib
    mk = os.path.join(CSRC, "Makefile")
    if not os.path.exists(mk):
        return None
    with open(mk) as f:
        line = next((x for x in f if x.startswith("HASHED =")), None)
    if line is None:
        return None
    h = hashlib.sha256()
    for name in line.split("=", 1)[1].split():
        with open(os.path.join(CSRC, name), "rb") as f:
            h.update(f.read())
    return h.hexdigest()[:16]


def _check_build(path, got):
    want = source_hash()
    got = got.decode() if got else ""
    if want is not None and got != want:
        raise ImportError(f"{path} was built from other sources (build id {got!r}, sources {want!r}): "
                          "run __graft_entry__.build()")


def load_run():
    global _run_lib
    if _run_lib is not None:
        return _run_lib
    load()
    if not os.path.exists(RUN_LIB_PATH):
        raise ImportError(f"{RUN_LIB_PATH} is missing: run __graft_entry__.build()")
    L = C.CDLL(RUN_LIB_PATH)
    L.ks_run_build_id.restype = C.c_char_p
    _check_build(RUN_LIB_PATH, L.ks_run_build_id())
    p = C.c_void_p
    L.ks_run.argtypes = [p, C.c_int64, C.c_int64, C.c_int32, p, p, p, C.c_int64, C.POINTER(C.c_int64),
                         C.POINTER(C.c_double)]
    L.ks_run.restype = C.c_int
    L.ks_trace_submit.argtypes = [p, C.c_int64, C.c_int64, p]
    L.ks_trace_submit.restype = C.c_int
    L.ks_local_exchange_create.argtypes = [C.c_int32]
    L.ks_local_exchange_create.restype = p
    L.ks_local_exchange_destroy.argtypes = [p]
    L.ks_local_exchange_destroy.restype = None
    L.ks_local_allgather.argtypes = [p, C.c_int32, C.c_int32, p, C.c_int64]
    L.ks_local_allgather.restype = C.c_int
    L.ks_local_exchange_abort.argtypes = [p]
    L.ks_local_exchange_abort.restype = None
    _run_lib = L
    return L


def load():
    global _lib
    if _lib is not None:
        return _lib
    if not os.path.exists(LIB_PATH):
        raise ImportError(f"{LIB_PATH} is missing: run __graft_entry__.build() (hipcc, gfx950)")
    L = C.CDLL(LIB_PATH)
    L.ks_build_id.restype = C.c_char_p
    _check_build(LIB_PATH, L.ks_build_id())
    p = C.c_void_p
    L.ks_create.argtypes = [C.POINTER(KsConfig), C.POINTER(C.c_void_p)]
    L.ks_create.restype = C.c_int
    L.ks_destroy.argtypes = [p]
    L.ks_destroy.restype = None
    L.ks_load_nodes.argtypes = [p, C.c_int64, p, p, p]
    L.ks_submit_pods.argtypes = [p, C.c_int64] + [p] * 10
    L.ks_step.argtypes = [p, C.c_int64, p, C.c_int64, C.POINTER(C.c_int64)]
    L.ks_filter.argtypes = [p, C.c_int64, p]
    L.ks_score.argtypes = [p, C.c_int64, p]
    L.ks_usage.argtypes = [p, p]
    L.ks_usage_at.argtypes = [p, C.c_int64, p]
    L.ks_usage_digest.argtypes = [p, C.c_int64, C.c_int64, p]
    L.ks_node_mix.argtypes = [C.c_int64]
    L.ks_node_mix.restype = C.c_uint64
# ... 88 lines not shown
```

kubernetes-simulator_amd/kubesim_amd/engine.py:

```python
from __future__ import annotations

import ctypes as C

import numpy as np

from . import _lib
from ._lib import KsBind, KsConfig, KsStepStats


class KsError(RuntimeError):
    def __init__(self, code: int, msg: str, binds=None):
        super().__init__(f"{_lib.STATUS_NAMES.get(code, code)}: {msg}")
        self.code = code
        self.kind = _lib.STATUS_NAMES.get(code, str(code))
        self.binds = binds


def _p(a):
    return a.ctypes.data_as(C.c_void_p)


def _c(a, dt):
    return np.ascontiguousarray(a, dtype=dt)


def _config(tick_seconds, filter_mode, filters, scorers, device, batch_pods, engine_flags):
    cfg = KsConfig()
    cfg.abi_version = _lib.KS_ABI_VERSION
    cfg.tick_seconds = tick_seconds
    cfg.filter_mode = filter_mode
    cfg.filters = filters
    cfg.n_scorers = len(scorers)
    for i, (k, w, v) in enumerate(scorers):
        cfg.scorers[i].kind, cfg.scorers[i].weight, cfg.scorers[i].value = k, w, v
    cfg.device = device
    cfg.batch_pods = batch_pods
    cfg.engine_flags = engine_flags
    return cfg


class Engine:
    def __init__(self, *, tick_seconds=10, filter_mode=_lib.KS_FILTER_REFERENCE_LITERAL, filters=0,
                 scorers=((_lib.KS_SCORER_CONST, 1, 1),), device=0, batch_pods=0, engine_flags=0,
                 _group=None):
        L = _lib.load()
        self._group = _group
        cfg = _config(tick_seconds, filter_mode, filters, scorers, device, batch_pods, engine_flags)
        h = C.c_void_p()
        if _group is None:
            rc = L.ks_create(C.byref(cfg), C.byref(h))
        else:
            rc = L.ks_group_add(_group.h, C.byref(cfg), C.byref(h))
        if rc != _lib.KS_OK:
            raise KsError(rc, "ks_create / ks_group_add rejected the configuration")
        self._L = L
        self.h = h
        self.n = 0
        self._submitted = 0

    def close(self):
        if getattr(self, "h", None):
            if getattr(self, "_group", None) is None:
                self._L.ks_destroy(self.h)
            self.h = None

    def __del__(self):
        self.close()

    def __enter__(self):
        return self

    def __exit__(self, *exc):
        self.close()

    def _check(self, rc, binds=None):
        if rc != _lib.KS_OK:
            raise KsError(rc, self._L.ks_last_error(self.h).decode(), binds)

    def shard(self, world: int, rank: int, comm_id: bytes | None = None, vshards: int = 1):
        buf = None
        if comm_id is not None:
            if len(comm_id) != _lib.KS_COMM_ID_BYTES:
                raise ValueError("comm_id must be KS_COMM_ID_BYTES long")
            buf = (C.c_uint8 * _lib.KS_COMM_ID_BYTES).from_buffer_copy(comm_id)
        self._check(self._L.ks_shard(self.h, world, rank, buf, vshards))

    def shard_host(self, world: int, rank: int, exchange: "LocalExchange", vshards: int = 1):
        self._xchg = exchange
        self._check(self._L.ks_shard_host(self.h, world, rank, vshards, exchange.fn, exchange.h))

    def load_nodes(self, alloc, taint, label):
        alloc = _c(alloc, np.int64).reshape(-1, 4)
        self.n = len(alloc)
        self._check(self._L.ks_load_nodes(self.h, self.n, _p(alloc), _p(_c(taint, np.uint64)),
                                          _p(_c(label, np.uint64))))

    def submit(self, pods: dict):
        m = int(pods["m"])
        arrs = [_c(pods["arrival"], np.int64), _c(pods["req"], np.int64).reshape(-1, 3),
                _c(pods["keymask"], np.uint8), _c(pods["tol"], np.uint64), _c(pods["sel"], np.uint64),
                _c(pods["phase_off"], np.int32), _c(pods["phase_sec"], np.int32),
                _c(pods["phase_use"], np.int64).reshape(-1, 3), _c(pods["flags"], np.uint8)]
        keys = pods.get("key_id")
        if keys is not None:
            keys = _c(keys, np.int64)
        per_pod = {"arrival": arrs[0], "req": arrs[1], "keymask": arrs[2], "tol": arrs[3], "sel": arrs[4],
                   "flags": arrs[8]}
        if keys is not None:
            per_pod["key_id"] = keys
        for name, a in per_pod.items():
            if len(a) != m:
                raise ValueError(f"pods[{name!r}] has {len(a)} rows, expected m = {m}")
        off = arrs[5]
        if len(off) != m + 1:
            raise ValueError(f"pods['phase_off'] has {len(off)} entries, expected m + 1 = {m + 1}")
        nf = int(off[-1]) if m else 0
        if m and (off[0] != 0 or (np.diff(off) < 0).any()):
            raise ValueError("pods['phase_off'] must start at 0 and be non-decreasing")
        if len(arrs[6]) < nf or len(arrs[7]) < nf:
            raise ValueError(f"phase arrays shorter than phase_off[-1] = {nf}")
        ptrs = [_p(a) for a in arrs] + [_p(keys) if keys is not None else None]
        self._check(self._L.ks_submit_pods(self.h, m, *ptrs))
        self._submitted += m

    def step(self, ticks: int, cap: int | None = None):
        if cap is None:
            cap = max(0, min(ticks, self.queued))
        out = (KsBind * max(cap, 1))()
        n = C.c_int64(0)
        rc = self._L.ks_step(self.h, ticks, out, cap, C.byref(n))
        k = min(n.value, cap)
        arr = np.frombuffer(out, dtype=np.dtype([("pod", "<i8"), ("node", "<i4"), ("status", "<i4"),
                                                 ("tick", "<i8")]), count=k).copy()
        self._check(rc, arr)
        return arr

    def filter(self, pod: int):
        mask = np.zeros(self.n, np.uint8)
        self._check(self._L.ks_filter(self.h, pod, _p(mask)))
        return mask

    def score(self, pod: int):
        score = np.zeros(self.n, np.int64)
        self._check(self._L.ks_score(self.h, pod, _p(score)))
        return score

    def usage(self):
        out = np.zeros((self.n, 3), np.int64)
        self._check(self._L.ks_usage(self.h, _p(out)))
        return out

    def usage_at(self, t: int):
        out = np.zeros((self.n, 3), np.int64)
        self._check(self._L.ks_usage_at(self.h, t, _p(out)))
        return out

    def usage_digest(self, t_lo: int, t_hi: int):
        out = np.zeros((max(t_hi - t_lo, 0), 6), np.uint64)
        self._check(self._L.ks_usage_digest(self.h, t_lo, t_hi, _p(out)))
        return out

    def requested_at(self, t: int):
        out = np.zeros((self.n, 4), np.int64)
        self._check(self._L.ks_requested_at(self.h, t, _p(out)))
        return out

    def filter_at(self, pod: int):
        mask = np.zeros(self.n, np.uint8)
        self._check(self._L.ks_filter_at(self.h, pod, _p(mask)))
        return mask

    def score_at(self, pod: int):
        score = np.zeros(self.n, np.int64)
        self._check(self._L.ks_score_at(self.h, pod, _p(score)))
        return score

    def cluster_series(self, t_lo: int, t_hi: int):
        out = np.zeros((max(t_hi - t_lo, 0), _lib.KS_SERIES_COLS), np.int64)
        self._check(self._L.ks_cluster_series(self.h, t_lo, t_hi, _p(out)))
        return out

    def node_peaks(self, t_lo: int, t_hi: int):
        out = np.zeros((self.n, 4), np.int64)
        self._check(self._L.ks_node_peaks(self.h, t_lo, t_hi, _p(out)))
        return out

    def pod_lookup(self, node: int, key_id: int):
        q = C.c_int64(-1)
        self._check(self._L.ks_pod_lookup(self.h, node, key_id, C.byref(q)))
        return q.value

    def node_pods(self, node: int):
        n = C.c_int64(0)
        self._check(self._L.ks_node_pods(self.h, node, None, 0, C.byref(n)))
# ... 150 lines not shown
```

Before: 90.73 billion evals/s.

## Skip speculative scan in single-GPU overlap path and load node records directly

In the single-GPU overlap path, the speculative per-batch scan launch is now skipped. Window prep marks a rescan case as an empty "fresh" window instead of rebuilding it. The merge kernel gains a direct mode that reads node constants from a new packed per-node table, filled by a new kernel before each step, and live usage from the SoA. It no longer reads staged e_rec copies, and the E-key build is deferred until after the list loads so the two can overlap. An opt-in SMALL_E flag lowers the E-set threshold that forces a rescan. The change adds an extra kernel launch per step and more scattered global reads in the merge, and relies on the fresh-window handshake being correct.

```diff
diff --git a/go/kubesim/engine/engine.go b/go/kubesim/engine/engine.go
--- a/go/kubesim/engine/engine.go
+++ b/go/kubesim/engine/engine.go
@@ -51,6 +51,7 @@
 const (
 	FlagNoOverlap   = uint32(C.KS_ENGINE_NO_OVERLAP)
 	FlagPrunedLists = uint32(C.KS_ENGINE_PRUNED_LISTS)
+	FlagSmallE      = uint32(C.KS_ENGINE_SMALL_E)
 )
 
 type ScorerSpec struct {
diff --git a/include/ks_engine.h b/include/ks_engine.h
--- a/include/ks_engine.h
+++ b/include/ks_engine.h
@@ -44,7 +44,8 @@
 
 enum { KS_ENGINE_FORCE_WIDE = 1, KS_ENGINE_NO_TINY = 2, KS_ENGINE_NO_MICRO = 4,
        KS_ENGINE_ONE_POD_RESOLVER = 8, KS_ENGINE_CHUNK_RESOLVER = 64, KS_ENGINE_NO_OVERLAP = 256,
-       KS_ENGINE_PRUNED_LISTS = 512 };
+       KS_ENGINE_PRUNED_LISTS = 512,
+       KS_ENGINE_SMALL_E = 2048 };
 
 typedef struct {
     int64_t pod;
diff --git a/kubernetes-simulator_amd/csrc/ks_cand.hip b/kubernetes-simulator_amd/csrc/ks_cand.hip
--- a/kubernetes-simulator_amd/csrc/ks_cand.hip
+++ b/kubernetes-simulator_amd/csrc/ks_cand.hip
@@ -53,7 +53,7 @@
 constexpr int kEPer = kEMax / 256;
 
 static_assert(kTopLOverlap >= kTopL, "merged lists kept at the longest list length");
-template <int kMode, int kLL>
+template <int kMode, int kLL, bool kDirect>
 __device__ __forceinline__ void cand_list(const EngineArgs& a, WinWS& ws, int i, const uint64_t* cand,
                                           const uint64_t* ek, int n_e) {
     static_assert(kLL >= kTopL && kLL <= kWave, "one list entry per lane");
@@ -108,8 +108,13 @@
         const uint64_t me = valid ? kept[lane] : 0ull;
         const int32_t nd = key_node(me);
         NodeV rec{};
+        uint4 rw[3] = {};
         int32_t eix = -1;
-        if (valid) { rec = load_node(a.s, nd); eix = a.e_idx[nd]; }
+        if (valid) {
+            if constexpr (kDirect) load_rec12c(a, nd, rw);
+            else rec = load_node(a.s, nd);
+            eix = a.e_idx[nd];
+        }
         if (valid && a.det_cids) atomicMin(&a.n_first[nd], i * kR + lane);
         int sl = valid ? atomicCAS(&a.n_slot[nd], -1, kSlotPending) : 0;
         const bool claim = valid && sl == -1;
@@ -124,7 +129,12 @@
             sl = base + __popcll(cm & ((1ull << lane) - 1ull));
             ws.slot_node[sl] = nd;
             if (sl < kSlotMax) {
-                put_rec(ws.slot_rec[sl], rec);
+                if constexpr (kDirect) {
+                    uint4* o = reinterpret_cast<uint4*>(ws.slot_rec[sl]);
+                    o[0] = rw[0]; o[1] = rw[1]; o[2] = rw[2];
+                } else {
+                    put_rec(ws.slot_rec[sl], rec);
+                }
                 ws.slot_eix[sl] = eix;
             }
             atomicExch(&a.n_slot[nd], sl);
@@ -155,7 +165,7 @@
 thread_local const EngineArgs* ks_mcl_host_args = nullptr;
 #endif
 namespace sq {
-template <int kMode, int kLL>
+template <int kMode, int kLL, bool kDirect>
 #ifdef KS_MCL_BYVAL
 __global__ __launch_bounds__(1024) void merge_cl_kernel(const EngineArgs av, const uint64_t* src,
                                                          int64_t pod_stride, int32_t nl, int64_t list_stride, int own_fb) {
@@ -196,36 +206,28 @@
 #pragma unroll
     for (int k = 0; k < kLL; ++k) top[k] = 0;
     const uint64_t* lists = src + (int64_t)(reuse ? 0 : sb) * pod_stride;
-    uint64_t lv0[kLL];
-    const bool has0 = tid < nfl;
-    {
-        const int l0 = has0 ? (pruned ? scn::flagged_block(tid, 0, nl, F) : tid) : 0;
-        const ulonglong2* lp = reinterpret_cast<const ulonglong2*>(lists + (int64_t)l0 * list_stride);
-#pragma unroll
-        for (int k = 0; k < kLL / 2; ++k) {
-            const ulonglong2 w = has0 ? lp[k] : make_ulonglong2(0, 0);
-            lv0[2 * k] = w.x;
-            lv0[2 * k + 1] = w.y;
-        }
-    }
     __shared__ uint64_t ek[kEMax];
-    const int n_e = ws.n_e;
-    {
-        const int64_t start = a.ctr[kCtrStart];
-        const int hi = ws.win_hi[b], n_es = ws.n_es;
-        uint4 er[2][3];
-        int32_t en[2], eu[2], ue[2];
+    const int n_e = ws.n_e, n_es = ws.n_es;
+    const int hi = ws.win_hi[b];
+    const int64_t start = a.ctr[kCtrStart];
+    uint4 er[2][3];
+    int32_t en[2], eu[2], ue[2];
+    auto e_index = [&]() {
 #pragma unroll
         for (int q = 0; q < 2; ++q) {
             const int k = tid + q * nthr;
             const int kc = k < kEMax ? k : kEMax - 1;
             const int ks = k < kWinSlots ? k : kWinSlots;
             en[q] = ws.e_node[kc];
-            const uint4* r = reinterpret_cast<const uint4*>(ws.e_rec[kc]);
-            er[q][0] = r[0]; er[q][1] = r[1]; er[q][2] = r[2];
+            if constexpr (!kDirect) {
+                const uint4* r = reinterpret_cast<const uint4*>(ws.e_rec[kc]);
+                er[q][0] = r[0]; er[q][1] = r[1]; er[q][2] = r[2];
+            }
             eu[q] = ws.e_off[ks];
             ue[q] = ws.e_off[ks < kWinSlots ? ks + 1 : ks];
         }
+    };
+    auto e_keys = [&]() {
 #if defined(KS_MCL_DIAG) && KS_MCL_DIAG == 2
         asm volatile("s_waitcnt vmcnt(0) lgkmcnt(0)" ::: "memory");
         uint64_t t_e0 = pstamp();
@@ -249,8 +251,13 @@
 #pragma unroll 1
         for (int k = tid + 2 * nthr; k < n_e; k += nthr) {
             const int32_t n = ws.e_node[k];
-            const uint4* r = reinterpret_cast<const uint4*>(ws.e_rec[k]);
-            const uint4 w3[3] = {r[0], r[1], r[2]};
+            uint4 w3[3];
+            if constexpr (kDirect) {
+                load_rec12c(a, n, w3);
+            } else {
+                const uint4* r = reinterpret_cast<const uint4*>(ws.e_rec[k]);
+                w3[0] = r[0]; w3[1] = r[1]; w3[2] = r[2];
+            }
             NodeV w = get_rec12(w3);
             const int ue1 = k < n_es ? ws.e_off[k + 1] : 0;
             for (int u = k < n_es ? ws.e_off[k] : 0; u < ue1; ++u) {
@@ -265,6 +272,27 @@
         if (tid == 0) { atomicAdd((unsigned long long*)&a.ctr[14], pstamp() - t_e0); atomicAdd((unsigned long long*)&a.ctr[24], (unsigned long long)(n_e > tid) + (n_e > tid + nthr)); }
         if (tid == 0) atomicAdd((unsigned long long*)&a.ctr[25], (unsigned long long)n_e);
 #endif
+    };
+    if constexpr (kDirect) e_index();
+    uint64_t lv0[kLL];
+    const bool has0 = tid < nfl;
+    {
+        const int l0 = has0 ? (pruned ? scn::flagged_block(tid, 0, nl, F) : tid) : 0;
+        const ulonglong2* lp = reinterpret_cast<const ulonglong2*>(lists + (int64_t)l0 * list_stride);
+#pragma unroll
+        for (int k = 0; k < kLL / 2; ++k) {
+            const ulonglong2 w = has0 ? lp[k] : make_ulonglong2(0, 0);
+            lv0[2 * k] = w.x;
+            lv0[2 * k + 1] = w.y;
+        }
+    }
+    if constexpr (kDirect) {
+#pragma unroll
+        for (int q = 0; q < 2; ++q)
+            load_rec12c(a, tid + q * nthr < n_e ? en[q] : 0, er[q]);
+    } else {
+        e_index();
+        e_keys();
     }
     if (has0) {
 #pragma unroll
@@ -295,6 +323,7 @@
         if (lane == 0) wl[wave][r] = m;
         if (hit && lane == __ffsll((unsigned long long)hit) - 1) head++;
     }
+    if constexpr (kDirect) e_keys();
     __syncthreads();
     PDG(MDG_AT(7, pt);)
     if (wave == 0 && nthr <= 256) {
@@ -337,7 +366,7 @@
     if (reuse) __syncthreads();
     if (tid < kLL) ws.mrg[mpar][b][tid] = pc[tid];
     PDG(MDG_AT(8, pt);)
-    cand_list<kMode, kLL>(a, ws, b, pc, ek, n_e);
+    cand_list<kMode, kLL, kDirect>(a, ws, b, pc, ek, n_e);
 }
 
 }
@@ -349,7 +378,8 @@
 }
 
 hipError_t launch_merge_cl(const EngineArgs* d, int mode, int B, const uint64_t* lists, int64_t pod_stride,
-                           int32_t nl, int64_t list_stride, int nl_max, hipStream_t st, int L, bool own_fallback) {
+                           int32_t nl, int64_t list_stride, int nl_max, hipStream_t st, int L, bool own_fallback,
+                           bool direct) {
     const int fb = own_fallback ? 1 : 0;
     static_assert(sq::kEPer * 256 >= kEMax, "E keys per thread at 256 threads");
     const dim3 g(B), t(nl_max > 1024 ? 1024 : 256);
@@ -358,16 +388,19 @@
     const EngineArgs hv = *ks_mcl_host_args;
 #define d hv
 #endif
-#define KS_MCL(LL)                                                                                                   \
+#define KS_MCL(LL, DR)                                                                                                   \
     switch (mode) {                                                                                                  \
-        case kEvalMicro: hipLaunchKernelGGL((sq::merge_cl_kernel<kEvalMicro, LL>), g, t, 0, st, d, lists, pod_stride, nl, list_stride, fb); break; \
-        case kEvalTiny: hipLaunchKernelGGL((sq::merge_cl_kernel<kEvalTiny, LL>), g, t, 0, st, d, lists, pod_stride, nl, list_stride, fb); break;   \
-        case kEvalNarrow: hipLaunchKernelGGL((sq::merge_cl_kernel<kEvalNarrow, LL>), g, t, 0, st, d, lists, pod_stride, nl, list_stride, fb); break; \
-        default: hipLaunchKernelGGL((sq::merge_cl_kernel<kEvalWide, LL>), g, t, 0, st, d, lists, pod_stride, nl, list_stride, fb); break;          \
-    }
-    if (L == kTopL) { KS_MCL(kTopL) }
-    else if (L == kTopLOverlap) { KS_MCL(kTopLOverlap) }
-    else return hipErrorInvalidValue;
+        case kEvalMicro: hipLaunchKernelGGL((sq::merge_cl_kernel<kEvalMicro, LL, DR>), g, t, 0, st, d, lists, pod_stride, nl, list_stride, fb); break; \
+        case kEvalTiny: hipLaunchKernelGGL((sq::merge_cl_kernel<kEvalTiny, LL, DR>), g, t, 0, st, d, lists, pod_stride, nl, list_stride, fb); break;   \
+        case kEvalNarrow: hipLaunchKernelGGL((sq::merge_cl_kernel<kEvalNarrow, LL, DR>), g, t, 0, st, d, lists, pod_stride, nl, list_stride, fb); break; \
+        default: hipLaunchKernelGGL((sq::merge_cl_kernel<kEvalWide, LL, DR>), g, t, 0, st, d, lists, pod_stride, nl, list_stride, fb); break;          \
+    }
+    if (L != kTopL && L != kTopLOverlap) return hipErrorInvalidValue;
+    if (direct) {
+        if (L == kTopL) { KS_MCL(kTopL, true) } else { KS_MCL(kTopLOverlap, true) }
+    } else {
+        if (L == kTopL) { KS_MCL(kTopL, false) } else { KS_MCL(kTopLOverlap, false) }
+    }
 #undef KS_MCL
 #ifdef KS_MCL_BYVAL
 #undef d
diff --git a/kubernetes-simulator_amd/csrc/ks_device.h b/kubernetes-simulator_amd/csrc/ks_device.h
--- a/kubernetes-simulator_amd/csrc/ks_device.h
+++ b/kubernetes-simulator_amd/csrc/ks_device.h
@@ -568,7 +568,8 @@
     uint32_t slot_rec[kSlotMax][kRecDw];
     int32_t touched[kTouchMax];
     int32_t n_touched, rescan;
-    int32_t lset, pad_;
+    int32_t lset;
+    int32_t fresh;
     int32_t split, moff, mpar, pad2_;
     uint64_t mrg[2][kWinMaxB][kTopLOverlap];
 #ifdef KS_BATCH_LOG
@@ -617,9 +618,26 @@
     int32_t nwl;
     int32_t lset;
     int32_t det_cids;
-    int32_t pad3_;
+    int32_t two_launch;
     const ScanRec* srec;
-};
+    const uint4* ncst;
+    int32_t e_lim;
+    int32_t pad4_;
+};
+constexpr int kSmallE = 128;
+static_assert(kSmallE <= kEMax, "E threshold within the arrays");
+__device__ __forceinline__ void load_rec12c(const EngineArgs& a, int32_t nd, uint4 (&w)[3]) {
+#ifdef KS_E_FROM_SOA
+    const NodeV v = load_node(a.s, nd);
+    w[0] = make_uint4((uint32_t)v.ac, (uint32_t)v.am, (uint32_t)v.ag, (uint32_t)(v.ap > 0x7FFFFFFF ? 0x7FFFFFFF : v.ap));
+    w[2] = make_uint4((uint32_t)v.taint, (uint32_t)(v.taint >> 32), (uint32_t)v.label, (uint32_t)(v.label >> 32));
+    w[1] = make_uint4((uint32_t)v.rc, (uint32_t)v.rm, (uint32_t)v.rg, (uint32_t)v.nr);
+#else
+    w[0] = a.ncst[2 * (int64_t)nd];
+    w[2] = a.ncst[2 * (int64_t)nd + 1];
+    w[1] = make_uint4((uint32_t)a.s.rc[nd], (uint32_t)a.s.rm[nd], (uint32_t)a.s.rg[nd], (uint32_t)a.s.nr[nd]);
+#endif
+}
 __host__ __device__ __forceinline__ uint64_t* lbit_of(const EngineArgs& a, int set, int b) {
     return a.lbit + ((int64_t)set * a.B + b) * a.nwl;
 }
@@ -650,7 +668,7 @@
 #endif
 hipError_t launch_merge_cl(const EngineArgs* d, int mode, int B, const uint64_t* lists, int64_t pod_stride,
                            int32_t nl, int64_t list_stride, int nl_max, hipStream_t st, int L = kTopL,
-                           bool own_fallback = false);
+                           bool own_fallback = false, bool direct = false);
 struct BindSeg {
     const int32_t* node;
     const int32_t* status;
@@ -658,6 +676,7 @@
 };
 hipError_t launch_gather_binds(const BindSeg* segs, int S, int64_t max_n, int32_t* node, int32_t* status,
                                hipStream_t st);
+hipError_t launch_node_consts(const NodeSoA& s, int64_t n_pad, uint4* out, hipStream_t st);
 hipError_t launch_rescale(const NodeSoA& s, int64_t n_pad, PodRec* pods, int64_t P, const int64_t f[3], hipStream_t st);
 
 struct CopySeg {
diff --git a/kubernetes-simulator_amd/csrc/ks_engine.cpp b/kubernetes-simulator_amd/csrc/ks_engine.cpp
--- a/kubernetes-simulator_amd/csrc/ks_engine.cpp
+++ b/kubernetes-simulator_amd/csrc/ks_engine.cpp
@@ -105,6 +105,7 @@
     int nwb = 0;
     bool nodes_loaded = false;
     void* node_mem = nullptr;
+    uint4* d_ncst = nullptr;
     ks::NodeSoA s{};
 
     DVec<ks::PodRec> pods;
@@ -259,6 +260,9 @@
     a.nwl = e->nwl;
     a.lset = 1;
     a.srec = e->srec.p;
+    a.ncst = e->d_ncst;
+    a.two_launch = 0;
+    a.e_lim = (e->flags & KS_ENGINE_SMALL_E) ? ks::kSmallE : ks::kEMax;
     return a;
 }
 
@@ -392,7 +396,7 @@
     if (cfg->batch_pods < 0 || cfg->batch_pods > kMaxBatch) return KS_EINVAL;
     if (cfg->engine_flags &
         ~(uint32_t)(KS_ENGINE_FORCE_WIDE | KS_ENGINE_NO_TINY | KS_ENGINE_NO_MICRO | KS_ENGINE_ONE_POD_RESOLVER |
-                    KS_ENGINE_CHUNK_RESOLVER | KS_ENGINE_NO_OVERLAP | KS_ENGINE_PRUNED_LISTS))
+                    KS_ENGINE_CHUNK_RESOLVER | KS_ENGINE_NO_OVERLAP | KS_ENGINE_PRUNED_LISTS | KS_ENGINE_SMALL_E))
         return KS_EINVAL;
     int64_t const_total = 0, w_lr = 0, w_ba = 0;
     for (int i = 0; i < cfg->n_scorers; i++) {
@@ -466,6 +470,7 @@
     e->preg.release(); e->d_blk.release(); e->d_digest.release(); e->srec.release();
     e->d_qs.release(); e->d_qi.release();
     if (e->node_mem) (void)hipFree(e->node_mem);
+    if (e->d_ncst) (void)hipFree(e->d_ncst);
     if (e->lists) (void)hipFree(e->lists);
     if (e->cand) (void)hipFree(e->cand);
     if (e->cand_all) (void)hipFree(e->cand_all);
@@ -623,6 +628,7 @@
     }
     HIPCHK(e, hipMalloc(&e->node_mem, sizeof(int64_t) * 10 * np));
     HIPCHK(e, hipMemcpyAsync(e->node_mem, h.data(), sizeof(int64_t) * 10 * np, hipMemcpyHostToDevice, e->st));
+    HIPCHK(e, hipMalloc(&e->d_ncst, sizeof(uint4) * 2 * np));
     int64_t* b = (int64_t*)e->node_mem;
     e->s.ac = b; e->s.am = b + np; e->s.ag = b + 2 * np; e->s.ap = b + 3 * np;
     e->s.rc = b + 4 * np; e->s.rm = b + 5 * np; e->s.rg = b + 6 * np; e->s.nr = b + 7 * np;
@@ -1191,9 +1197,12 @@
     const int which = resolver_of(e);
     const bool fused = which == kResolveChunk;
     HIPCHK(e, hipMemcpyAsync(e->d_ctr, e->h_ctr, 5 * sizeof(int64_t), hipMemcpyHostToDevice, st));
-    HIPCHK(e, hipMemcpyAsync(e->d_args, e->h_args, sizeof(ks::EngineArgs), hipMemcpyHostToDevice, st));
     const bool overlap = fused && e->overlap && e->d_args_spec && key16(e) && e->blk_n <= kOverlapMaxBlocks;
     const bool pipe = fused && !overlap && e->overlap && e->st2 && e->world * e->vsh > 1;
+    const bool two = overlap && e->world * e->vsh == 1;
+    e->h_args->two_launch = two ? 1 : 0;
+    HIPCHK(e, hipMemcpyAsync(e->d_args, e->h_args, sizeof(ks::EngineArgs), hipMemcpyHostToDevice, st));
+    if (two) HIPCHK(e, ks::launch_node_consts(e->s, e->n_pad, e->d_ncst, st));
     e->L = (overlap && e->world * e->vsh == 1 && !e->prune) || pipe ? ks::kTopLOverlap : ks::kTopL;
     if (pipe) {
         *e->h_args_full = *e->h_args;
@@ -1242,13 +1251,14 @@
             if (ev[0]) HIPCHK(e, hipEventRecord(ev[0], st));
             if (!spec) HIPCHK(e, fused ? ks::launch_window_prep(d, true, false, (int)(b & 1), st) : ks::launch_expire_head(d, 1, st));
             if (ev[1]) HIPCHK(e, hipEventRecord(ev[1], st));
-            HIPCHK(e, ks::launch_scan(d, 1, e->blk_n, e->B, e->PG, e->mode, key16(e), st, spec, e->prune, e->L, fused));
+            const bool scan = !(two && spec);
+            if (scan) HIPCHK(e, ks::launch_scan(d, 1, e->blk_n, e->B, e->PG, e->mode, key16(e), st, spec, e->prune, e->L, fused && !two));
             if (ev[2]) HIPCHK(e, hipEventRecord(ev[2], st));
             const int G = e->world * e->vsh;
             hipEvent_t evx[2] = {ev[5], ev[6]};
             const int64_t L = ks::kTopL, BL = (int64_t)e->B * L;
             if (G == 1) {
-                HIPCHK(e, fused ? ks::launch_merge_cl(d, e->mode, e->B, nullptr, 0, 0, 0, e->nblk, st, e->L)
+                HIPCHK(e, fused ? ks::launch_merge_cl(d, e->mode, e->B, nullptr, 0, 0, 0, e->nblk, st, e->L, false, two)
                                 : ks::launch_merge(d, 1, e->B, nullptr, 0, 0, 0, nullptr, e->nblk, st));
             } else {
                 HIPCHK(e, part_merges(e, d, st, -1));
@@ -1265,7 +1275,7 @@
             else
                 HIPCHK(e, fused ? ks::launch_chunk_only(d, e->mode, st) : launch_resolver(d, 1, e->mode, which, st));
             if (ev[4]) HIPCHK(e, hipEventRecord(ev[4], st));
-            if (e->profiling) kind.push_back((uint8_t)((!spec ? 1 : 0) | (overlap && b + 1 < nbat ? 2 : 0) | (G > 1 ? 4 : 0)));
+            if (e->profiling) kind.push_back((uint8_t)((!spec ? 1 : 0) | (overlap && b + 1 < nbat ? 2 : 0) | (G > 1 ? 4 : 0) | (scan ? 16 : 0)));
             launches++;
         }
         HIPCHK(e, hipMemcpyAsync(e->h_ctr, e->d_ctr, 5 * sizeof(int64_t), hipMemcpyDeviceToHost, st));
@@ -1326,7 +1336,7 @@
             scan_ms += t[1];
             res_ms += t[3];
             ks.prep_ms += t[0]; ks.prep_n += kind[l] & 1;
-            ks.scan_ms += t[1]; ks.scan_n += 1;
+            ks.scan_ms += t[1]; ks.scan_n += kind[l] & 16 ? 1 : 0;
             ks.merge_ms += t[2]; ks.merge_n += 1;
             if (kind[l] & 2) { ks.fused_ms += t[3]; ks.fused_n += 1; }
             else { ks.resolve_ms += t[3]; ks.resolve_n += 1; }
diff --git a/kubernetes-simulator_amd/csrc/ks_kernels.hip b/kubernetes-simulator_amd/csrc/ks_kernels.hip
--- a/kubernetes-simulator_amd/csrc/ks_kernels.hip
+++ b/kubernetes-simulator_amd/csrc/ks_kernels.hip
@@ -1047,6 +1047,22 @@
     return hipGetLastError();
 }
 
+__global__ __launch_bounds__(256) void node_consts_kernel(const NodeSoA s, int64_t n_pad, uint4* __restrict__ out) {
+    const int64_t i = (int64_t)blockIdx.x * blockDim.x + threadIdx.x;
+    if (i >= n_pad) return;
+    const int64_t ap = s.ap[i];
+    const uint64_t t = s.taint[i], l = s.label[i];
+    out[2 * i] = make_uint4((uint32_t)s.ac[i], (uint32_t)s.am[i], (uint32_t)s.ag[i],
+                            (uint32_t)(ap > 0x7FFFFFFF ? 0x7FFFFFFF : ap));
+    out[2 * i + 1] = make_uint4((uint32_t)t, (uint32_t)(t >> 32), (uint32_t)l, (uint32_t)(l >> 32));
+}
+
+hipError_t launch_node_consts(const NodeSoA& s, int64_t n_pad, uint4* out, hipStream_t st) {
+    if (n_pad <= 0) return hipSuccess;
+    hipLaunchKernelGGL(node_consts_kernel, dim3((unsigned)((n_pad + 255) / 256)), dim3(256), 0, st, s, n_pad, out);
+    return hipGetLastError();
+}
+
 hipError_t launch_rescale(const NodeSoA& s, int64_t n_pad, PodRec* pods, int64_t P, const int64_t f[3], hipStream_t st) {
     hipLaunchKernelGGL(rescale_kernel, dim3(1024), dim3(256), 0, st, s, n_pad, pods, P, f[0], f[1], f[2]);
     return hipGetLastError();
diff --git a/kubernetes-simulator_amd/csrc/ks_prep.h b/kubernetes-simulator_amd/csrc/ks_prep.h
--- a/kubernetes-simulator_amd/csrc/ks_prep.h
+++ b/kubernetes-simulator_amd/csrc/ks_prep.h
@@ -51,7 +51,7 @@
     int nb = (int)min<int64_t>(min<int64_t>(a.B, kWinMaxB), end - start);
     if (err != 0 || nb <= 0) {
         if (tid == 0) {
-            ws.nb = 0; ws.e_cnt = 0; ws.n_e = 0; ws.n_es = 0; ws.rescan = 0; ws.lset = 1;
+            ws.nb = 0; ws.e_cnt = 0; ws.n_e = 0; ws.n_es = 0; ws.rescan = 0; ws.lset = 1; ws.fresh = 0;
             ws.split = 0; ws.moff = 0; ws.mpar = slot;
             spec_out[kCtrStart] = end; spec_out[kCtrEnd] = end; spec_out[kCtrErr] = 0; spec_out[kSpecPrev] = start;
         }
@@ -63,8 +63,9 @@
     const int64_t mypos = tid < nb ? a.exp_pos[start + tid] : 0;
     const int64_t sp_start = spec ? spec_in[kCtrStart] : 0;
     const int64_t prev_start = spec ? spec_in[kSpecPrev] : 0;
-    const int n_touched = spec ? ws.n_touched : 0;
-    const int n_eold = spec ? ws.n_e : 0;
+    const bool fresh = spec && a.two_launch && ws.fresh != 0;
+    const int n_touched = spec && !fresh ? ws.n_touched : 0;
+    const int n_eold = spec && !fresh ? ws.n_e : 0;
     constexpr int kOPer = (kEMax + NT - 1) / NT;
     int32_t eold[kOPer];
 #pragma unroll
@@ -88,9 +89,10 @@
     const int e_cnt = (int)(L.off[nb - 1] - e_base);
     const bool reuse = spec && start != sp_start && start > prev_start && start < sp_start;
     int rescan = 0;
-    if (spec) rescan = (start != sp_start && !reuse) ||
-                       (int64_t)e_cnt + (e1 - e0) + n_touched + (reuse ? n_eold : 0) > kEMax;
-    const bool touch = spec && !rescan;
+    if (spec && !fresh) rescan = (start != sp_start && !reuse) ||
+                                 (int64_t)e_cnt + (e1 - e0) + n_touched + (reuse ? n_eold : 0) > a.e_lim;
+    const bool touch = spec && !rescan && !fresh;
+    const bool empty = rescan && a.two_launch;
     const int32_t hq = head && tid < e1 - e0 ? a.exp_pod[e0 + tid] : -1;
     const int32_t wq = tid < e_cnt ? a.exp_pod[e_base + tid] : -1;
     int32_t hst = 1, hex = 1, hnd = 0, wst = 1, wex = 1, wnd = 0;
@@ -127,6 +129,15 @@
             if (touch) L.xn[atomicAdd(&L.s_nx, 1)] = nd;
         }
     }
+    if (empty) {
+        if (tid == 0) {
+            ws.nb = 0; ws.e_cnt = 0; ws.n_e = 0; ws.n_es = 0; ws.nslot = 0; ws.rescan = 0; ws.lset = 0; ws.fresh = 1;
+            ws.split = 0; ws.moff = 0; ws.mpar = slot;
+            a.ctr[kCtrRescan] += 1;
+            spec_out[kCtrStart] = start; spec_out[kCtrEnd] = end; spec_out[kCtrErr] = 0; spec_out[kSpecPrev] = start;
+        }
+        return;
+    }
     if (touch) {
 #pragma unroll
         for (int q = 0; q < kTPer; ++q)
@@ -223,7 +234,8 @@
     for (int k = tid; k < n_e; k += NT) a.e_idx[ws.e_node[k]] = k;
     if (tid == 0) {
         ws.nb = nb; ws.e_cnt = e_cnt; ws.n_e = n_e; ws.n_es = n_es; ws.nslot = 0; ws.rescan = rescan;
-        ws.lset = touch ? 0 : 1;
+        ws.lset = touch || fresh ? 0 : 1;
+        ws.fresh = 0;
         if (rescan) a.ctr[kCtrRescan] += 1;
         if (touch && reuse) a.ctr[kCtrReuse] += 1;
         ws.split = touch && reuse ? (int32_t)(sp_start - start) : 0;
diff --git a/kubernetes-simulator_amd/kubesim_amd/_lib.py b/kubernetes-simulator_amd/kubesim_amd/_lib.py
--- a/kubernetes-simulator_amd/kubesim_amd/_lib.py
+++ b/kubernetes-simulator_amd/kubesim_amd/_lib.py
@@ -21,6 +21,7 @@
 KS_ENGINE_CHUNK_RESOLVER = 64
 KS_ENGINE_NO_OVERLAP = 256
 KS_ENGINE_PRUNED_LISTS = 512
+KS_ENGINE_SMALL_E = 2048
 KS_SELFTEST_LR_MICRO = 0
 KS_SERIES_COLS = 7
 
diff --git a/kubernetes-simulator_amd/kubesim_amd/engine.py b/kubernetes-simulator_amd/kubesim_amd/engine.py
--- a/kubernetes-simulator_amd/kubesim_amd/engine.py
+++ b/kubernetes-simulator_amd/kubesim_amd/engine.py
@@ -40,6 +40,7 @@
 
 
 class Engine:
+
     def __init__(self, *, tick_seconds=10, filter_mode=_lib.KS_FILTER_REFERENCE_LITERAL, filters=0,
                  scorers=((_lib.KS_SCORER_CONST, 1, 1),), device=0, batch_pods=0, engine_flags=0,
                  _group=None):
```

Measured after the change: 93.30 billion evals/s (median of 6 runs). 2.8% higher.
